# marco-conciatori-public/weed_instance_segmentation

Measured on AMD Instinct MI355X. Metric: images/sec at 1024x1024 bs=8 per GPU (Mask2Former R50, 100 queries, fp32 forward-only), higher is better.
Workload: dtype f32

## Files before the change

include/wm2f.h:

```cpp
#ifndef WM2F_H
#define WM2F_H

#include <stdint.h>

#ifdef __cplusplus
extern "C" {
#endif

#define WM2F_VERSION 100

#define WM2F_F32 0
#define WM2F_BF16 1
#define WM2F_I32 2
#define WM2F_U8 3
#define WM2F_U16 4
#define WM2F_I64 5

#define WM2F_OK 0
#define WM2F_EINVAL (-1)
#define WM2F_EUNSUPPORTED (-2)
#define WM2F_ELAUNCH (-3)

#define WM2F_MAX_LEVELS 8

int wm2f_version(void);
const char* wm2f_last_error(void);

int wm2f_msdeform_fwd(const void* value, const void* loc, const void* attn_w, void* out,
                      const int32_t* level_hw, int B, int S, int Q, int heads, int D, int L, int P,
                      int dtype, void* stream);

int wm2f_msdeform_bwd(const void* value, const void* loc, const void* attn_w, const void* grad_out,
                      void* grad_value, void* grad_loc, void* grad_attn_w,
                      const int32_t* level_hw, int B, int S, int Q, int heads, int D, int L, int P,
                      int dtype, void* stream);

int64_t wm2f_msdeform_bwd_det_workspace(const int32_t* level_hw, int B, int S, int heads, int D, int L);
int wm2f_msdeform_bwd_det(const void* value, const void* loc, const void* attn_w, const void* grad_out,
                          void* grad_value, void* grad_loc, void* grad_attn_w, void* workspace,
                          const int32_t* level_hw, int B, int S, int Q, int heads, int D, int L, int P, int dtype,
                          void* stream);

int wm2f_msdeform_rows_fwd(const void* value, const void* rows, void* out, const int32_t* level_hw, int B, int S, int Q,
                           int heads, int D, int L, int P, int dtype, void* stream);
int wm2f_msdeform_rows_bwd(const void* value, const void* rows, const void* grad_out, void* grad_value, void* grad_rows,
                           const int32_t* level_hw, int B, int S, int Q, int heads, int D, int L, int P, int dtype,
                           void* stream);

int wm2f_msdeform_fused_fwd(const void* value, const void* offsets, const void* logits, const void* ref,
                            void* out, const int32_t* level_hw, int B, int S, int Q, int heads, int D,
                            int L, int P, int dtype, void* stream);

int wm2f_msdeform_fused_packed_fwd(const void* value, const void* packed, void* out,
                                   const int32_t* level_hw, int B, int S, int Q, int heads, int D, int L,
                                   int P, int dtype, int margin, void* stream);

int wm2f_msdeform_fused_lanes_fwd(const void* value, const void* lanes, void* out, const int32_t* level_hw, int B, int S,
                                  int Q, int heads, int D, int L, int P, int dtype, int head_major, void* stream);

int wm2f_msdeform_fwd_v(const void* value, const void* a, const void* b, const void* ref, void* out,
                        const int32_t* level_hw, int B, int S, int Q, int heads, int D, int L, int P,
                        int dtype, int fused, int variant, int margin, void* stream);

int wm2f_mask_einsum_bf16_fwd(const void* emb, const void* pix_pixel_major, void* out, int B, int Q, int C,
                              int HW, void* stream);

int64_t wm2f_mask_einsum_bf16_bwd_workspace(int B, int Q, int C, int HW);
int wm2f_mask_einsum_bf16_bwd(const void* emb, const void* pix, const void* grad_out, void* g_emb, void* g_pix,
                              void* workspace, int B, int Q, int C, int HW, void* stream);
int wm2f_nchw_to_pixel_major_bf16(const void* src, void* dst, int B, int C, int HW, void* stream);

int wm2f_mask_einsum_fwd(const void* emb, const void* pix, void* out, int B, int Q, int C, int HW,
                         int dtype, void* stream);

int wm2f_mask_einsum_attn_mask_fwd(const void* emb, const void* pix, void* mask, void* row_open, int B, int Q, int C,
                                   int HW, int dtype, void* stream);

int64_t wm2f_mask_einsum_bwd_workspace(int B, int Q, int C, int HW);
int wm2f_mask_einsum_bwd(const void* emb, const void* pix, const void* grad_out, void* g_emb, void* g_pix,
                         void* workspace, int B, int Q, int C, int HW, int dtype, void* stream);

int wm2f_attn_mask_build(const void* logits, void* mask, void* row_open, int B, int Q, int H, int W,
                         int Hn, int Wn, void* stream);

int64_t wm2f_masked_xattn_workspace(int B, int heads, int Q, int N, int D);
int wm2f_masked_xattn_fwd(const void* q, const void* k, const void* v, const void* mask,
                          const void* row_open, void* out, void* lse, void* workspace,
                          int B, int heads, int Q, int N, int D, int dtype, void* stream);

int wm2f_masked_xattn_bf16_fwd(const void* q, const void* k, const void* v, const void* mask, const void* row_open,
                               void* out, void* lse, void* workspace, int B, int heads, int Q, int N, int D, void* stream);

int64_t wm2f_masked_xattn_bwd_workspace(int B, int heads, int Q, int N, int D);
int wm2f_masked_xattn_bwd(const void* q, const void* k, const void* v, const void* mask,
                          const void* row_open, const void* out, const void* lse, const void* grad_out,
                          void* grad_q, void* grad_k, void* grad_v, void* workspace,
                          int B, int heads, int Q, int N, int D, int dtype, void* stream);

int wm2f_masked_xattn_bf16_bwd(const void* q, const void* k, const void* v, const void* mask, const void* row_open,
                               const void* out, const void* lse, const void* grad_out, void* grad_q, void* grad_k,
                               void* grad_v, void* workspace, int B, int heads, int Q, int N, int D, void* stream);

#define WM2F_K2_UNSUPPORTED 0
#define WM2F_K2_FWD_GENERAL 1
#define WM2F_K2_FWD_FULL 2
#define WM2F_K2_BF16_FWD 3
#define WM2F_K2_BWD_GENERAL 4
#define WM2F_K2_BWD_FULL 5
#define WM2F_K2_BF16_BWD 6
int wm2f_masked_xattn_route(int B, int heads, int Q, int N, int D, int dtype, int backward, int mask_aligned, int* route);

int wm2f_swin_window_attn_fwd(const void* q, const void* k, const void* v, const void* k_pad, const void* v_pad,
                              const void* bias_table, void* out, int B, int H, int W, int heads, int D, int ws, int shift,
                              int dtype, void* stream);

int wm2f_swin_window_attn_train_fwd(const void* q, const void* k, const void* v, const void* k_pad, const void* v_pad,
                                    const void* bias_table, void* out, void* lse, int B, int H, int W, int heads, int D, int ws,
                                    int shift, int dtype, void* stream);
int64_t wm2f_swin_window_attn_bwd_workspace(int B, int H, int W, int heads, int D, int ws);
int wm2f_swin_window_attn_bwd(const void* q, const void* k, const void* v, const void* k_pad, const void* v_pad,
                              const void* bias_table, const void* lse, const void* grad_out, void* grad_q, void* grad_k,
                              void* grad_v, void* grad_k_pad, void* grad_v_pad, void* grad_bias_table, void* workspace, int B,
                              int H, int W, int heads, int D, int ws, int shift, int dtype, void* stream);

int64_t wm2f_matcher_workspace(int NL, int B, int Q, int P, int Tsum);
int wm2f_matcher_cost(const void* mask_logits, const void* class_logits, const void* tgt_masks,
                      int tgt_dtype, const int32_t* tgt_offset, const void* tgt_classes,
                      const void* points, void* cost, void* workspace, int NL, int B, int Q, int C1,
                      int h, int w, int Ht, int Wt, int P, int Tmax, float w_class, float w_mask,
                      float w_dice, void* stream);
int wm2f_matcher_cost_levels(const void* const* mask_levels, const void* class_logits, const void* tgt_masks,
                             int tgt_dtype, const int32_t* tgt_offset, const void* tgt_classes,
                             const void* points, void* cost, void* workspace, int NL, int B, int Q, int C1, int h,
                             int w, int Ht, int Wt, int P, int Tmax, float w_class, float w_mask, float w_dice,
                             void* stream);

int wm2f_lsa_batched(const void* cost, const void* counts, void* rows, void* cols, int problems, int B, int Q, int Tmax, int Tcap,
                     void* stream);

int wm2f_point_sample_fwd(const void* feat, int feat_dtype, const void* pts, const void* map_index,
                          void* out, int M, int H, int W, int P, void* stream);
int wm2f_point_sample_bwd(const void* grad_out, const void* pts, const void* map_index, void* grad_feat,
                          int M, int H, int W, int P, void* stream);

int wm2f_add_broadcast(const void* a, const void* p, void* out, int B, int64_t n, void* stream);
int wm2f_bias_act(const void* x, const void* bias, const void* residual, void* y, int N, int C, int HW,
                  int relu, void* stream);
int wm2f_add_layernorm(const void* x, const void* residual, const void* gamma, const void* beta,
                       const void* pos, void* out, void* out_plus_pos, int64_t rows, int C,
                       int64_t pos_rows, float eps, void* stream);
int64_t wm2f_add_layernorm_train_workspace(int64_t rows);
int wm2f_add_layernorm_train_fwd(const void* x, int x_dtype, const void* residual, const void* gamma, const void* beta,
                                 const void* pos, void* y, void* y_bf16, void* y_plus_pos, int yp_dtype, void* stats,
                                 int64_t rows, int C, int64_t pos_rows, float eps, float clamp, void* stream);
int wm2f_add_layernorm_train_bwd(const void* x, int x_dtype, const void* residual, const void* gamma, const void* stats,
                                 const void* grad_y, const void* grad_y_bf16, const void* grad_y_plus_pos, int gyp_dtype,
                                 void* grad_sum, void* grad_x, void* grad_gamma, void* grad_beta, void* workspace,
                                 int64_t rows, int C, void* stream);
int wm2f_token_linear_fwd(const void* x, const void* w, const void* bias, const void* residual, const void* ln_gamma,
                          const void* ln_beta, const void* pos, void* out, void* out_plus_pos, int64_t M, int K, int N, int relu,
                          int64_t pos_rows, float eps, int out_group, void* stream);

int wm2f_token_linear_split_weight(const void* w, void* w_split, int N, int K, void* stream);
int wm2f_token_linear_split_fwd(const void* x, const void* w_split, const void* bias, const void* residual, const void* ln_gamma,
                                const void* ln_beta, const void* pos, void* out, void* out_plus_pos, int64_t M, int K, int N,
                                int relu, int64_t pos_rows, float eps, int out_group, void* stream);

int wm2f_conv1x1_split_fwd(const void* x, const void* w_split, const void* bias, const void* residual, void* out, int B, int K,
                           int N, int Hi, int Wi, int stride, int relu, int config, void* stream);
int wm2f_conv1x1_split_config(int N, int P, int B, int n_cu);

int wm2f_conv3x3_split_fwd(const void* x, const void* w_split, const void* bias, void* out, int B, int Cin, int N, int Hi,
                           int Wi, int stride, int relu, int config, void* stream);
int wm2f_conv3x3_split_config(int N, int P, int B, int n_cu);

int wm2f_stem7x7_pool_fwd(const void* x, const void* w_split, const void* bias, void* out, int B, int Cin, int N, int Hi,
                          int Wi, int grid, void* stream);

int64_t wm2f_token_wgrad_workspace(int64_t M, int N, int K);
int wm2f_token_wgrad_bf16(const void* dy, const void* x, void* dw, void* db, void* workspace, int64_t M, int N, int K,
                          void* stream);
int wm2f_token_wgrad_f32(const void* dy, const void* x, void* dw, void* db, void* workspace, int64_t M, int N, int K,
                         void* stream);
int wm2f_tokens_to_nchw(const void* tokens, void* out, int B, int S, int C, int start, int HW, void* stream);
int wm2f_group_norm_tokens(const void* x, const void* bias, const void* gamma, const void* beta, void* tokens,
                           void* stats_ws, int B, int C, int G, int HW, int S, int start, float eps, void* stream);
int wm2f_resize_bilinear(const void* x, void* y, int NC, int H, int W, int Ho, int Wo, void* stream);
int wm2f_resize_pyramid(const void* x, void* y2, void* y4, void* y8, int NC, int H, int W, void* stream);
int wm2f_bias_relu_maxpool(const void* x, const void* bias, void* y, int N, int C, int H, int W, void* stream);
int wm2f_group_norm_act(const void* x, const void* gamma, const void* beta, const void* up, void* y, void* stats_ws,
                        int B, int C, int G, int H, int W, int Hs, int Ws, float eps, int relu, void* stream);

int wm2f_select_top_points(const void* score, const void* pts, void* out, int rows, int n, int k, int out_row_points,
                           void* stream);

int wm2f_point_sample_levels_fwd(const void* const* level_maps, int n_levels, const void* pts, const int32_t* index,
                                 void* out, int M, int H, int W, int P, int neg_abs, void* stream);
int wm2f_point_sample_levels_bwd(const void* grad_out, const void* pts, const int32_t* index,
                                 void* const* level_grads, int n_levels, int M, int H, int W, int P, void* stream);
int wm2f_point_sample_levels_bwd_unique(const void* grad_out, const void* pts, const int32_t* index,
                                        void* const* level_grads, int n_levels, int M, int H, int W, int P, void* stream);
int wm2f_mask_loss_rows_fwd(const void* logits, const void* labels, void* sums, void* bce_mean, void* dice,
                            int R, int P, void* stream);
int wm2f_mask_loss_rows_bwd(const void* logits, const void* labels, const void* sums, const void* g_bce,
                            const void* g_dice, void* grad, int R, int P, void* stream);

int wm2f_instance_scores(const void* mask_logits, const int32_t* qidx, void* sum_sig, void* cnt, int B, int Q,
                         int K, int h, int w, int gh, int gw, void* stream);
int wm2f_instance_any(const void* mask_logits, const int32_t* qidx, const uint8_t* cand, int32_t* any_out, int B,
                      int Q, int K, int h, int w, int gh, int gw, int Ho, int Wo, void* stream);
int wm2f_instance_segmentation(const void* mask_logits, const int32_t* kept_q, const int32_t* n_kept,
                               void* segmentation, int B, int Q, int K, int h, int w, int gh, int gw, int Ho,
                               int Wo, void* stream);
int wm2f_instance_maps(const void* image_logits, const int32_t* kept_q, int n, void* maps, int h, int w, int gh,
                       int gw, int Ho, int Wo, void* stream);

int wm2f_semantic_scores(const void* mask_logits, const void* class_probs, void* scores, int B, int Q, int C, int h,
                         int w, int gh, int gw, void* stream);
int wm2f_semantic_resize_argmax(const void* scores, const int32_t* rows, int nrows, void* segmentation,
                                void* out_scores, int C, int gh, int gw, int Ho, int Wo, void* stream);
int wm2f_panoptic_probs(const void* mask_logits, const int32_t* kept_q, const int32_t* n_kept, void* probs, int B,
                        int Q, int K, int h, int w, int gh, int gw, void* stream);
int wm2f_panoptic_segments(const void* probs, const int32_t* rows, const int32_t* n_kept, const void* scores,
                           int32_t* segmentation, int32_t* counts, int nrows, int K, int gh, int gw, int Ho, int Wo,
                           float mask_threshold, void* stream);
int wm2f_panoptic_relabel(int32_t* segmentation, const int32_t* rows, const int32_t* table, int nrows, int K,
                          int64_t n_pixels, void* stream);

int wm2f_labelmap_to_masks(const int32_t* label_map, const int32_t* ids, uint8_t* masks, int64_t n_pixels, int T,
                           void* stream);

int wm2f_labelmap_pair_counts(const void* pred_map, int pred_dtype, const void* gt_map, int gt_dtype,
                              const int32_t* gt_ids, const int32_t* n_ids, int32_t* hist, int B, int64_t n_pixels, int P,
                              int G, void* stream);
int64_t wm2f_mask_pair_counts_workspace(int D, int G, int64_t n_pixels);
int wm2f_mask_pair_counts(const uint8_t* det_masks, const uint8_t* gt_masks, int32_t* inter, int32_t* det_area,
                          int32_t* gt_area, void* workspace, int D, int G, int64_t n_pixels, void* stream);
int wm2f_coco_match(const int32_t* inter, const int32_t* det_area, const int32_t* gt_area, const int32_t* det_label,
                    const int32_t* gt_label, const int32_t* det_order, const int32_t* n_det, const int32_t* n_gt,
                    const double* iou_thresholds, const double* area_ranges, int32_t* det_rank, uint8_t* det_matched,
                    uint8_t* det_ignored, uint8_t* gt_ignored, int B, int D, int G, int T, int A, int max_det,
                    void* stream);
int wm2f_coco_match_min(const int32_t* inter, const int32_t* det_area, const int32_t* gt_area, const int32_t* inter2,
                        const int32_t* det_area2, const int32_t* gt_area2, const int32_t* det_label,
                        const int32_t* gt_label, const int32_t* det_order, const int32_t* n_det, const int32_t* n_gt,
                        const double* iou_thresholds, const double* area_ranges, int32_t* det_rank,
                        uint8_t* det_matched, uint8_t* det_ignored, uint8_t* gt_ignored, int B, int D, int G, int T,
                        int A, int max_det, void* stream);

int wm2f_labelmap_instance_stats(const void* map, int dtype, const int32_t* ids, const int32_t* n_ids, int64_t* stats,
                                 int B, int H, int W, int N, void* stream);

int64_t wm2f_labelmap_boundary_workspace(int B, int H, int W);
int wm2f_labelmap_boundary(const void* map, int dtype, int32_t* out, void* workspace, int B, int H, int W, int d,
                           void* stream);

int wm2f_panoptic_match(const int32_t* hist, const int32_t* pred_label, const int32_t* gt_label, const int32_t* n_pred,
                        const int32_t* n_gt, int32_t* gt_match, double* gt_iou, uint8_t* pred_state, int B, int P, int G,
                        int void_as_background, void* stream);
int wm2f_semantic_confusion(const void* pred, int pred_dtype, const void* gt, int gt_dtype, const int32_t* gt_ids,
                            const int32_t* gt_cls, const int32_t* n_ids, int64_t* conf, int64_t* n_out_of_range, int B,
                            int64_t n_pixels, int G, int C, int ignore_index, int background_label, void* stream);

int wm2f_labelmap_overlay(const uint8_t* image, const void* map, int dtype, const int32_t* ids, const int32_t* n_ids,
                          const uint8_t* rgba, const int32_t* order, uint32_t default_rgba, int inner, int outer,
                          uint8_t* out, int B, int H, int W, int N, void* stream);

#define WM2F_PRE_MAX_IMAGES 32
#define WM2F_PRE_MAX_SIDE 16384
#define WM2F_PRE_DESC_LEN 12
#define WM2F_LAB_DESC_LEN 7
int wm2f_resize_normalize_u8(const uint8_t* images, int64_t images_bytes, const int64_t* desc, const int32_t* tables,
                             int64_t n_table, const float* lut, uint8_t* workspace, int64_t workspace_bytes,
                             float* pixel_values, int64_t* pixel_mask, int B, int Hp, int Wp, void* stream);
int wm2f_resize_nearest_labels(const void* maps, int dtype, int64_t n_map_elems, const int64_t* desc,
                               const int32_t* tables, int64_t n_table, int32_t* out, uint8_t* present, int B, int Hp,
                               int Wp, int ignore_index, void* stream);

#define WM2F_AUG_MAX_VIRTUAL 65536
#define WM2F_AUG_PRE_DESC_LEN 16
#define WM2F_AUG_LAB_DESC_LEN 12
int wm2f_augment_resize_normalize_u8(const uint8_t* images, int64_t images_bytes, const int64_t* desc,
                                     const int32_t* tables, int64_t n_table, const float* lut, float* pixel_values,
                                     int64_t* pixel_mask, int B, int Hp, int Wp, void* stream);
int wm2f_augment_nearest_labels(const void* maps, int dtype, int64_t n_map_elems, const int64_t* desc,
                                const int32_t* tables, int64_t n_table, int32_t* out, uint8_t* present, int B, int Hp,
                                int Wp, int ignore_index, void* stream);

#define WM2F_PHOTO_BRIGHTNESS 0
#define WM2F_PHOTO_CONTRAST 1
#define WM2F_PHOTO_SATURATION 2
#define WM2F_PHOTO_HUE 3
#define WM2F_PHOTO_DESC_LEN 12
int64_t wm2f_photometric_workspace(int B);
int wm2f_photometric_u8(uint8_t* images, int64_t images_bytes, const int64_t* desc, void* workspace, int B, void* stream);

#define WM2F_CCL_VALUE 0
#define WM2F_CCL_BINARY 1
#define WM2F_CCL_RGB 2
#define WM2F_CCL_MAX_COLORS 16
int64_t wm2f_ccl_workspace(int H, int W);
int wm2f_ccl_label(const void* src, int mode, int src_dtype, int src_H, int src_W, const int32_t* ty, const int32_t* tx,
                   const uint8_t* colors, int n_colors, int H, int W, void* workspace, int32_t* count, void* stream);
int wm2f_ccl_keys(const void* workspace, int n, int H, int W, int64_t* keys, void* stream);
int wm2f_ccl_paint(void* workspace, const int64_t* order, int n, int H, int W, int skip_255, int background, int32_t* out,
                   int32_t* comp_class, void* stream);
int wm2f_resize_nearest(const void* src, int elem_bytes, int src_H, int src_W, const int32_t* ty, const int32_t* tx,
                        void* dst, int H, int W, void* stream);

#define WM2F_POLY_MAX_SIDE 16384
#define WM2F_POLY_MAX_COORD (1 << 24)
int64_t wm2f_poly_workspace(int H, int W, int n_verts);
int wm2f_poly_fill(int32_t* out, int H, int W, const int32_t* verts, int n_verts, const int32_t* contour_offsets,
                   int n_contours, const int32_t* call_offsets, const int32_t* values, const int32_t* call_row0,
                   const int32_t* item_offsets, int n_calls, int n_items, void* workspace, void* stream);

#define WM2F_RLE_MAX_IDS 1024
int64_t wm2f_rle_workspace(int B, int H, int W, int N, int order);
int wm2f_labelmap_toggle_counts(const void* map, int dtype, int32_t* counts, int32_t* out_of_range, void* workspace,
                                int B, int H, int W, int N, int order, void* stream);
int wm2f_labelmap_toggles(const void* map, int dtype, const int32_t* offsets, int32_t* positions, void* workspace, int B,
                          int H, int W, int N, int order, void* stream);
int64_t wm2f_rle_paint_workspace(int B, int H, int W);
int wm2f_rle_paint(int32_t* out, const int32_t* runs, int R, int32_t* status, void* workspace, int B, int H, int W,
                   int order, void* stream);

int64_t wm2f_trace_workspace(int B, int H, int W, int N);
int64_t wm2f_trace_edge_workspace(int64_t E);
int wm2f_trace_rounds(int64_t E);
int wm2f_trace_count(const void* map, int dtype, int32_t* counts, void* workspace, int B, int H, int W, int N,
                     void* stream);
int wm2f_trace_link(const void* map, int dtype, const void* workspace, void* edge_workspace, int E, int B, int H, int W,
                    int N, void* stream);
int wm2f_trace_rank(void* edge_workspace, int E, void* stream);
int wm2f_trace_flags(const void* edge_workspace, int32_t* flag, int32_t* lead, int E, int H, int W, int coords,
                     int simplify, void* stream);
int wm2f_trace_loops(const void* map, int dtype, const void* edge_workspace, const int32_t* lead_prefix,
                     int64_t* loop_key, int32_t* loop_len, int E, int n_loops, int B, int H, int W, int N, void* stream);
int wm2f_trace_scatter(const void* edge_workspace, const int32_t* flag, const int32_t* lead_prefix,
                       const int32_t* loop_place, const int32_t* loop_base, int32_t* flag_sorted, int32_t* edge_sorted,
                       int32_t* term_sorted, int E, int n_loops, int H, int W, void* stream);
int wm2f_trace_emit(const void* edge_workspace, const int32_t* flag_sorted, const int32_t* edge_sorted,
                    const int32_t* flag_prefix, int32_t* points, int E, int P, int H, int W, int coords, void* stream);

#define WM2F_TILE_MAX_SIDE 16384
#define WM2F_TILE_MAX_IDS 256
#define WM2F_TILE_MAX_TILES 1024
#define WM2F_TILE_MAX_PAIRS 16384
int64_t wm2f_tile_merge_workspace(int T, int N, int P);
int wm2f_tile_pair_counts(const void* tiles, int dtype, const int32_t* n_ids, const int32_t* pairs, int32_t* hist, int T,
                          int th, int tw, int N, int P, void* stream);
int wm2f_tile_owned_counts(const void* tiles, int dtype, const int32_t* n_ids, const int32_t* geom, int32_t* owned, int T,
                           int th, int tw, int N, void* stream);
int wm2f_tile_link(const int32_t* hist, const int32_t* pairs, const int32_t* labels, const int32_t* n_ids,
                   const int32_t* owned, int32_t* remap, int32_t* n_merged, void* workspace, int T, int N, int P, int num,
                   int den, void* stream);
int wm2f_tile_compose(const void* tiles, int dtype, const int32_t* n_ids, const int32_t* geom, const int32_t* remap,
                      int32_t* out, int T, int th, int tw, int N, int H, int W, void* stream);

#ifdef __cplusplus
}
#endif
#endif
```

weed_instance_segmentation_amd/_lib.py:

```python
from __future__ import annotations

import ctypes
import os
from ctypes import POINTER, c_char_p, c_float, c_int, c_int32, c_int64, c_void_p

HERE = os.path.dirname(os.path.abspath(__file__))
LIB_PATH = os.path.join(HERE, "libwm2f.so")
PROF_LIB_PATH = os.path.join(HERE, "libwm2f_prof.so")
if os.environ.get("WM2F_PROF_LIB"):
    PROF_LIB_PATH = os.environ["WM2F_PROF_LIB"]

WM2F_F32 = 0
WM2F_BF16 = 1
WM2F_I32 = 2
WM2F_U8 = 3
WM2F_U16 = 4
WM2F_I64 = 5
WM2F_CCL_VALUE, WM2F_CCL_BINARY, WM2F_CCL_RGB = 0, 1, 2
WM2F_CCL_MAX_COLORS = 16
WM2F_POLY_MAX_SIDE = 16384
WM2F_POLY_MAX_COORD = 1 << 24
WM2F_RLE_MAX_IDS = 1024
WM2F_AUG_MAX_VIRTUAL = 65536
WM2F_TILE_MAX_SIDE, WM2F_TILE_MAX_IDS, WM2F_TILE_MAX_TILES, WM2F_TILE_MAX_PAIRS = 16384, 256, 1024, 16384
WM2F_AUG_PRE_DESC_LEN, WM2F_AUG_LAB_DESC_LEN = 16, 12
WM2F_PHOTO_BRIGHTNESS, WM2F_PHOTO_CONTRAST, WM2F_PHOTO_SATURATION, WM2F_PHOTO_HUE = 0, 1, 2, 3
WM2F_PHOTO_DESC_LEN = 12
(WM2F_K2_UNSUPPORTED, WM2F_K2_FWD_GENERAL, WM2F_K2_FWD_FULL, WM2F_K2_BF16_FWD, WM2F_K2_BWD_GENERAL, WM2F_K2_BWD_FULL,
 WM2F_K2_BF16_BWD) = range(7)
WM2F_OK, WM2F_EINVAL, WM2F_EUNSUPPORTED, WM2F_ELAUNCH = 0, -1, -2, -3

_P = c_void_p
_I = c_int
_HOST_I32 = POINTER(c_int32)

SIGNATURES = {
    "wm2f_version": (c_int, []),
    "wm2f_last_error": (c_char_p, []),
    "wm2f_msdeform_fwd": (c_int, [_P, _P, _P, _P, _HOST_I32, _I, _I, _I, _I, _I, _I, _I, _I, _P]),
    "wm2f_msdeform_bwd": (c_int, [_P, _P, _P, _P, _P, _P, _P, _HOST_I32, _I, _I, _I, _I, _I, _I, _I, _I, _P]),
    "wm2f_msdeform_rows_fwd": (c_int, [_P, _P, _P, _HOST_I32, _I, _I, _I, _I, _I, _I, _I, _I, _P]),
    "wm2f_msdeform_rows_bwd": (c_int, [_P, _P, _P, _P, _P, _HOST_I32, _I, _I, _I, _I, _I, _I, _I, _I, _P]),
    "wm2f_msdeform_bwd_det_workspace": (c_int64, [_HOST_I32, _I, _I, _I, _I, _I]),
    "wm2f_msdeform_bwd_det": (c_int, [_P, _P, _P, _P, _P, _P, _P, _P, _HOST_I32, _I, _I, _I, _I, _I, _I, _I, _I, _P]),
    "wm2f_msdeform_fused_fwd": (c_int, [_P, _P, _P, _P, _P, _HOST_I32, _I, _I, _I, _I, _I, _I, _I, _I, _P]),
    "wm2f_msdeform_fused_packed_fwd": (c_int, [_P, _P, _P, _HOST_I32, _I, _I, _I, _I, _I, _I, _I, _I, _I, _P]),
    "wm2f_msdeform_fused_lanes_fwd": (c_int, [_P, _P, _P, _HOST_I32, _I, _I, _I, _I, _I, _I, _I, _I, _I, _P]),
    "wm2f_msdeform_fwd_v": (c_int, [_P, _P, _P, _P, _P, _HOST_I32, _I, _I, _I, _I, _I, _I, _I, _I, _I, _I, _I, _P]),
    "wm2f_select_top_points": (c_int, [_P, _P, _P, _I, _I, _I, _I, _P]),
    "wm2f_point_sample_levels_fwd": (c_int, [POINTER(c_void_p), _I, _P, _P, _P, _I, _I, _I, _I, _I, _P]),
    "wm2f_point_sample_levels_bwd": (c_int, [_P, _P, _P, POINTER(c_void_p), _I, _I, _I, _I, _I, _P]),
    "wm2f_point_sample_levels_bwd_unique": (c_int, [_P, _P, _P, POINTER(c_void_p), _I, _I, _I, _I, _I, _P]),
    "wm2f_mask_loss_rows_fwd": (c_int, [_P, _P, _P, _P, _P, _I, _I, _P]),
    "wm2f_mask_loss_rows_bwd": (c_int, [_P, _P, _P, _P, _P, _P, _I, _I, _P]),
    "wm2f_labelmap_to_masks": (c_int, [_P, _P, _P, c_int64, _I, _P]),
    "wm2f_instance_scores": (c_int, [_P, _P, _P, _P, _I, _I, _I, _I, _I, _I, _I, _P]),
    "wm2f_instance_any": (c_int, [_P, _P, _P, _P, _I, _I, _I, _I, _I, _I, _I, _I, _I, _P]),
    "wm2f_instance_segmentation": (c_int, [_P, _P, _P, _P, _I, _I, _I, _I, _I, _I, _I, _I, _I, _P]),
    "wm2f_instance_maps": (c_int, [_P, _P, _I, _P, _I, _I, _I, _I, _I, _I, _P]),
    "wm2f_semantic_scores": (c_int, [_P, _P, _P, _I, _I, _I, _I, _I, _I, _I, _P]),
    "wm2f_semantic_resize_argmax": (c_int, [_P, _P, _I, _P, _P, _I, _I, _I, _I, _I, _P]),
    "wm2f_panoptic_probs": (c_int, [_P, _P, _P, _P, _I, _I, _I, _I, _I, _I, _I, _P]),
    "wm2f_panoptic_segments": (c_int, [_P, _P, _P, _P, _P, _P, _I, _I, _I, _I, _I, _I, c_float, _P]),
    "wm2f_panoptic_relabel": (c_int, [_P, _P, _P, _I, _I, c_int64, _P]),
    "wm2f_mask_einsum_bf16_fwd": (c_int, [_P, _P, _P, _I, _I, _I, _I, _P]),
    "wm2f_nchw_to_pixel_major_bf16": (c_int, [_P, _P, _I, _I, _I, _P]),
    "wm2f_mask_einsum_fwd": (c_int, [_P, _P, _P, _I, _I, _I, _I, _I, _P]),
    "wm2f_mask_einsum_attn_mask_fwd": (c_int, [_P, _P, _P, _P, _I, _I, _I, _I, _I, _P]),
    "wm2f_mask_einsum_bf16_bwd_workspace": (c_int64, [_I, _I, _I, _I]),
    "wm2f_mask_einsum_bf16_bwd": (c_int, [_P, _P, _P, _P, _P, _P, _I, _I, _I, _I, _P]),
    "wm2f_mask_einsum_bwd_workspace": (c_int64, [_I, _I, _I, _I]),
    "wm2f_mask_einsum_bwd": (c_int, [_P, _P, _P, _P, _P, _P, _I, _I, _I, _I, _I, _P]),
    "wm2f_attn_mask_build": (c_int, [_P, _P, _P, _I, _I, _I, _I, _I, _I, _P]),
    "wm2f_masked_xattn_workspace": (c_int64, [_I, _I, _I, _I, _I]),
    "wm2f_masked_xattn_fwd": (c_int, [_P, _P, _P, _P, _P, _P, _P, _P, _I, _I, _I, _I, _I, _I, _P]),
    "wm2f_masked_xattn_route": (c_int, [_I, _I, _I, _I, _I, _I, _I, _I, _HOST_I32]),
    "wm2f_masked_xattn_bf16_fwd": (c_int, [_P, _P, _P, _P, _P, _P, _P, _P, _I, _I, _I, _I, _I, _P]),
    "wm2f_masked_xattn_bf16_bwd": (c_int, [_P, _P, _P, _P, _P, _P, _P, _P, _P, _P, _P, _P, _I, _I, _I, _I, _I, _P]),
    "wm2f_masked_xattn_bwd_workspace": (c_int64, [_I, _I, _I, _I, _I]),
    "wm2f_masked_xattn_bwd": (c_int, [_P, _P, _P, _P, _P, _P, _P, _P, _P, _P, _P, _P, _I, _I, _I, _I, _I, _I, _P]),
    "wm2f_swin_window_attn_fwd": (c_int, [_P, _P, _P, _P, _P, _P, _P, _I, _I, _I, _I, _I, _I, _I, _I, _P]),
    "wm2f_swin_window_attn_train_fwd": (c_int, [_P, _P, _P, _P, _P, _P, _P, _P, _I, _I, _I, _I, _I, _I, _I, _I, _P]),
    "wm2f_swin_window_attn_bwd_workspace": (c_int64, [_I, _I, _I, _I, _I, _I]),
    "wm2f_swin_window_attn_bwd": (c_int, [_P] * 15 + [_I] * 8 + [_P]),
    "wm2f_matcher_workspace": (c_int64, [_I, _I, _I, _I, _I]),
    "wm2f_matcher_cost": (c_int, [_P, _P, _P, _I, _HOST_I32, _P, _P, _P, _P, _I, _I, _I, _I, _I, _I, _I, _I, _I, _I,
                                  c_float, c_float, c_float, _P]),
    "wm2f_matcher_cost_levels": (c_int, [POINTER(c_void_p), _P, _P, _I, _HOST_I32, _P, _P, _P, _P, _I, _I, _I, _I, _I, _I, _I,
                                         _I, _I, _I, c_float, c_float, c_float, _P]),
    "wm2f_lsa_batched": (c_int, [_P, _P, _P, _P, _I, _I, _I, _I, _I, _P]),
    "wm2f_add_broadcast": (c_int, [_P, _P, _P, _I, c_int64, _P]),
    "wm2f_bias_act": (c_int, [_P, _P, _P, _P, _I, _I, _I, _I, _P]),
    "wm2f_add_layernorm": (c_int, [_P, _P, _P, _P, _P, _P, _P, c_int64, _I, c_int64, c_float, _P]),
    "wm2f_add_layernorm_train_workspace": (c_int64, [c_int64]),
    "wm2f_add_layernorm_train_fwd": (c_int, [_P, _I, _P, _P, _P, _P, _P, _P, _P, _I, _P, c_int64, _I, c_int64, c_float, c_float, _P]),
    "wm2f_add_layernorm_train_bwd": (c_int, [_P, _I, _P, _P, _P, _P, _P, _P, _I, _P, _P, _P, _P, _P, c_int64, _I, _P]),
    "wm2f_token_linear_fwd": (c_int, [_P, _P, _P, _P, _P, _P, _P, _P, _P, c_int64, _I, _I, _I, c_int64, c_float, _I, _P]),
    "wm2f_token_linear_split_weight": (c_int, [_P, _P, _I, _I, _P]),
    "wm2f_token_linear_split_fwd": (c_int, [_P, _P, _P, _P, _P, _P, _P, _P, _P, c_int64, _I, _I, _I, c_int64, c_float, _I, _P]),
    "wm2f_conv1x1_split_config": (c_int, [_I, _I, _I, _I]),
    "wm2f_conv1x1_split_fwd": (c_int, [_P, _P, _P, _P, _P, _I, _I, _I, _I, _I, _I, _I, _I, _P]),
    "wm2f_conv3x3_split_config": (c_int, [_I, _I, _I, _I]),
    "wm2f_conv3x3_split_fwd": (c_int, [_P, _P, _P, _P, _I, _I, _I, _I, _I, _I, _I, _I, _P]),
    "wm2f_stem7x7_pool_fwd": (c_int, [_P, _P, _P, _P, _I, _I, _I, _I, _I, _I, _P]),
    "wm2f_token_wgrad_workspace": (c_int64, [c_int64, _I, _I]),
    "wm2f_token_wgrad_bf16": (c_int, [_P, _P, _P, _P, _P, c_int64, _I, _I, _P]),
    "wm2f_token_wgrad_f32": (c_int, [_P, _P, _P, _P, _P, c_int64, _I, _I, _P]),
    "wm2f_tokens_to_nchw": (c_int, [_P, _P, _I, _I, _I, _I, _I, _P]),
    "wm2f_group_norm_tokens": (c_int, [_P, _P, _P, _P, _P, _P, _I, _I, _I, _I, _I, _I, c_float, _P]),
    "wm2f_resize_bilinear": (c_int, [_P, _P, _I, _I, _I, _I, _I, _P]),
    "wm2f_resize_pyramid": (c_int, [_P, _P, _P, _P, _I, _I, _I, _P]),
    "wm2f_bias_relu_maxpool": (c_int, [_P, _P, _P, _I, _I, _I, _I, _P]),
    "wm2f_group_norm_act": (c_int, [_P, _P, _P, _P, _P, _P, _I, _I, _I, _I, _I, _I, _I, c_float, _I, _P]),
    "wm2f_point_sample_fwd": (c_int, [_P, _I, _P, _P, _P, _I, _I, _I, _I, _P]),
    "wm2f_point_sample_bwd": (c_int, [_P, _P, _P, _P, _I, _I, _I, _I, _P]),
    "wm2f_labelmap_pair_counts": (c_int, [_P, _I, _P, _I, _P, _P, _P, _I, c_int64, _I, _I, _P]),
    "wm2f_mask_pair_counts_workspace": (c_int64, [_I, _I, c_int64]),
    "wm2f_mask_pair_counts": (c_int, [_P, _P, _P, _P, _P, _P, _I, _I, c_int64, _P]),
    "wm2f_coco_match": (c_int, [_P] * 14 + [_I, _I, _I, _I, _I, _I, _P]),
    "wm2f_coco_match_min": (c_int, [_P] * 17 + [_I, _I, _I, _I, _I, _I, _P]),
    "wm2f_labelmap_boundary_workspace": (c_int64, [_I, _I, _I]),
    "wm2f_labelmap_boundary": (c_int, [_P, _I, _P, _P, _I, _I, _I, _I, _P]),
    "wm2f_labelmap_instance_stats": (c_int, [_P, _I, _P, _P, _P, _I, _I, _I, _I, _P]),
    "wm2f_panoptic_match": (c_int, [_P] * 8 + [_I, _I, _I, _I, _P]),
    "wm2f_semantic_confusion": (c_int, [_P, _I, _P, _I, _P, _P, _P, _P, _P, _I, c_int64, _I, _I, _I, _I, _P]),
    "wm2f_labelmap_overlay": (c_int, [_P, _P, _I, _P, _P, _P, _P, ctypes.c_uint32, _I, _I, _P, _I, _I, _I, _I, _P]),
    "wm2f_resize_normalize_u8": (c_int, [_P, c_int64, POINTER(c_int64), _P, c_int64, _P, _P, c_int64, _P, _P, _I, _I, _I,
                                         _P]),
    "wm2f_resize_nearest_labels": (c_int, [_P, _I, c_int64, POINTER(c_int64), _P, c_int64, _P, _P, _I, _I, _I, _I, _P]),
    "wm2f_augment_resize_normalize_u8": (c_int, [_P, c_int64, POINTER(c_int64), _P, c_int64, _P, _P, _P, _I, _I, _I, _P]),
    "wm2f_augment_nearest_labels": (c_int, [_P, _I, c_int64, POINTER(c_int64), _P, c_int64, _P, _P, _I, _I, _I, _I, _P]),
    "wm2f_photometric_workspace": (c_int64, [_I]),
    "wm2f_photometric_u8": (c_int, [_P, c_int64, POINTER(c_int64), _P, _I, _P]),
    "wm2f_ccl_workspace": (c_int64, [_I, _I]),
    "wm2f_ccl_label": (c_int, [_P, _I, _I, _I, _I, _P, _P, POINTER(ctypes.c_uint8), _I, _I, _I, _P, _P, _P]),
    "wm2f_ccl_keys": (c_int, [_P, _I, _I, _I, _P, _P]),
    "wm2f_ccl_paint": (c_int, [_P, _P, _I, _I, _I, _I, _I, _P, _P, _P]),
    "wm2f_resize_nearest": (c_int, [_P, _I, _I, _I, _P, _P, _P, _I, _I, _P]),
    "wm2f_poly_workspace": (c_int64, [_I, _I, _I]),
    "wm2f_poly_fill": (c_int, [_P, _I, _I, _P, _I, _P, _I, _P, _P, _P, _P, _I, _I, _P, _P]),
    "wm2f_rle_workspace": (c_int64, [_I, _I, _I, _I, _I]),
    "wm2f_labelmap_toggle_counts": (c_int, [_P, _I, _P, _P, _P, _I, _I, _I, _I, _I, _P]),
    "wm2f_labelmap_toggles": (c_int, [_P, _I, _P, _P, _P, _I, _I, _I, _I, _I, _P]),
    "wm2f_rle_paint_workspace": (c_int64, [_I, _I, _I]),
    "wm2f_rle_paint": (c_int, [_P, _P, _I, _P, _P, _I, _I, _I, _I, _P]),
    "wm2f_trace_workspace": (c_int64, [_I, _I, _I, _I]),
    "wm2f_trace_edge_workspace": (c_int64, [c_int64]),
    "wm2f_trace_rounds": (c_int, [c_int64]),
    "wm2f_trace_count": (c_int, [_P, _I, _P, _P, _I, _I, _I, _I, _P]),
    "wm2f_trace_link": (c_int, [_P, _I, _P, _P, _I, _I, _I, _I, _I, _P]),
    "wm2f_trace_rank": (c_int, [_P, _I, _P]),
    "wm2f_trace_flags": (c_int, [_P, _P, _P, _I, _I, _I, _I, _I, _P]),
    "wm2f_trace_loops": (c_int, [_P, _I, _P, _P, _P, _P, _I, _I, _I, _I, _I, _I, _P]),
    "wm2f_trace_scatter": (c_int, [_P, _P, _P, _P, _P, _P, _P, _P, _I, _I, _I, _I, _P]),
    "wm2f_trace_emit": (c_int, [_P, _P, _P, _P, _P, _I, _I, _I, _I, _I, _P]),
    "wm2f_tile_merge_workspace": (c_int64, [_I, _I, _I]),
    "wm2f_tile_pair_counts": (c_int, [_P, _I, _P, _P, _P, _I, _I, _I, _I, _I, _P]),
    "wm2f_tile_owned_counts": (c_int, [_P, _I, _P, _P, _P, _I, _I, _I, _I, _P]),
    "wm2f_tile_link": (c_int, [_P, _P, _P, _P, _P, _P, _P, _P, _I, _I, _I, _I, _I, _P]),
    "wm2f_tile_compose": (c_int, [_P, _I, _P, _P, _P, _P, _I, _I, _I, _I, _I, _I, _P]),
}

PROF_SIGNATURES = {"wm2f_debug_stamps": (c_int, [_P, c_int64])}

_lib = None


class Wm2fError(RuntimeError):
    pass


def use_profiling_library() -> ctypes.CDLL:
    global _lib
    if _lib is not None:
        raise Wm2fError("use_profiling_library() must come before the first kernel call")
    if not os.path.exists(PROF_LIB_PATH):
        raise Wm2fError(f"{PROF_LIB_PATH} not found: python -m weed_instance_segmentation_amd._build --prof")
    lib = ctypes.CDLL(PROF_LIB_PATH)
    for name, (res, args) in {**SIGNATURES, **PROF_SIGNATURES}.items():
        fn = getattr(lib, name)
        fn.restype, fn.argtypes = res, args
    _lib = lib
    return lib


def load() -> ctypes.CDLL:
    global _lib
    if _lib is None:
        if not os.path.exists(LIB_PATH):
            raise Wm2fError(
                f"{LIB_PATH} not found: build it with `python -m weed_instance_segmentation_amd._build` "
                "(hipcc, gfx950). There is no CPU or PyTorch fallback for the hot path.")
        lib = ctypes.CDLL(LIB_PATH)
        for name, (res, args) in SIGNATURES.items():
            fn = getattr(lib, name)
            fn.restype = res
            fn.argtypes = args
        _lib = lib
    return _lib


def check(rc: int, what: str) -> None:
    if rc != 0:
        msg = load().wm2f_last_error()
        raise Wm2fError(f"{what} failed (code {rc}): {msg.decode() if msg else '?'}")


def host_i32(values) -> ctypes.Array:
    flat = [int(v) for v in values]
    return (c_int32 * len(flat))(*flat)
```

weed_instance_segmentation_amd/csrc/conv1x1_split.hip:

```cpp
#include "common.h"

namespace wm2f {
namespace {

using f32x4 = __attribute__((ext_vector_type(4))) float;
using f32x8 = __attribute__((ext_vector_type(8))) float;
using bf16x8 = __attribute__((ext_vector_type(8))) __bf16;
typedef __attribute__((address_space(3))) void* lds_ptr_t;

constexpr int kWaves = 8;
constexpr int kThreads = kWaves * 64;
constexpr int kCT = 2;
constexpr int kKStep = 32;
constexpr int kFrag = 1024;
constexpr unsigned kOob = 0x80000000u;
constexpr float kBf16Max = 3.38953139e38f;

enum : int { kRaw = 0, kBias = 1, kBiasRelu = 2, kBiasResRelu = 3 };

__device__ __forceinline__ void split3(const f32x8 x, bf16x8& h, bf16x8& m, bf16x8& l) {
  f32x8 xc;
#pragma unroll
  for (int i = 0; i < 8; ++i) xc[i] = __builtin_amdgcn_fmed3f(x[i], -kBf16Max, kBf16Max);
  h = __builtin_convertvector(xc, bf16x8);
  const f32x8 r1 = x - __builtin_convertvector(h, f32x8);
  m = __builtin_convertvector(r1, bf16x8);
  const f32x8 r2 = r1 - __builtin_convertvector(m, f32x8);
  l = __builtin_convertvector(r2, bf16x8);
}

struct C1Args {
  const float *x, *bias, *residual;
  const void* ws;
  float* out;
  int K, N;
  int Hi, Wi, Wo, P, stride;
};

__device__ __forceinline__ void c1_barrier() {
  asm volatile("s_waitcnt vmcnt(0)" ::: "memory");
  __builtin_amdgcn_s_barrier();
  asm volatile("" ::: "memory");
}

template <int NRT, int WN, int EPI>
__global__ __launch_bounds__(kThreads) void conv1x1_split_kernel(C1Args a) {
  extern __shared__ __attribute__((aligned(16))) unsigned char smem[];
  constexpr int kRowTiles = WN * NRT;
  constexpr int kPanelBytes = kRowTiles * 3 * kFrag;
  constexpr int kPieces = kRowTiles * 3;
  constexpr int kPT = (kWaves / WN) * kCT * 16;
  const int tid = threadIdx.x, lane = tid & 63, wave = __builtin_amdgcn_readfirstlane(tid >> 6);
  const int wn = wave % WN, wp = wave / WN;
  const int g = lane >> 4, j = lane & 15;
  const int nb = blockIdx.x, b = blockIdx.z;
  const int n_wg = nb * kRowTiles * 16;
  const int p_w = blockIdx.y * kPT + wp * kCT * 16;
  const int n_ks = a.K / kKStep;
  const int HWi = a.Hi * a.Wi;

  const __amdgpu_buffer_rsrc_t w_rs = __builtin_amdgcn_make_buffer_rsrc((void*)a.ws, 0, a.N * a.K * 6, 0x00020000);
  const __amdgpu_buffer_rsrc_t x_rs =
      __builtin_amdgcn_make_buffer_rsrc((void*)(a.x + (int64_t)b * a.K * HWi), 0, a.K * HWi * 4, 0x00020000);

  unsigned xo[kCT];
#pragma unroll
  for (int c = 0; c < kCT; ++c) {
    const int p = p_w + c * 16 + j;
    const int ho = p / a.Wo, wo = p - ho * a.Wo;
    xo[c] = p < a.P ? (unsigned)(((8 * g) * HWi + a.stride * (ho * a.Wi + wo)) * 4) : kOob;
  }
  const unsigned ch_bytes = (unsigned)HWi * 4;

  f32x8 xr[kCT];
  auto issue = [&](int ks) {
    unsigned char* dst = smem + (ks & 1) * kPanelBytes;
    const int src = (ks * (a.N / 16) + n_wg / 16) * 3 * kFrag;
    for (int f = wave; f < kPieces; f += kWaves)
      __builtin_amdgcn_raw_ptr_buffer_load_lds(w_rs, (lds_ptr_t)(dst + f * kFrag), 16, lane * 16, src + f * kFrag, 0, 0);
    const unsigned kb = (unsigned)(ks * kKStep) * ch_bytes;
#pragma unroll
    for (int c = 0; c < kCT; ++c) {
      const unsigned o = xo[c] == kOob ? kOob : xo[c] + kb;
#pragma unroll
      for (int i = 0; i < 8; ++i)
        xr[c][i] = __builtin_bit_cast(float, __builtin_amdgcn_raw_buffer_load_b32(x_rs, o, i * ch_bytes, 0));
    }
  };

  issue(0);
  c1_barrier();

  f32x4 acc[NRT][kCT];
#pragma unroll
  for (int rt = 0; rt < NRT; ++rt)
#pragma unroll
    for (int c = 0; c < kCT; ++c) acc[rt][c] = (f32x4){0.f, 0.f, 0.f, 0.f};

  for (int ks = 0; ks < n_ks; ++ks) {
    bf16x8 bh[kCT], bm[kCT], bl[kCT];
#pragma unroll
    for (int c = 0; c < kCT; ++c) split3(xr[c], bh[c], bm[c], bl[c]);
    if (ks + 1 < n_ks) issue(ks + 1);

    const unsigned char* panel = smem + (ks & 1) * kPanelBytes + wn * NRT * 3 * kFrag;
    auto read_a = [&](bf16x8 (&dst)[3], int rt) {
#pragma unroll
      for (int p = 0; p < 3; ++p) dst[p] = *reinterpret_cast<const bf16x8*>(panel + (rt * 3 + p) * kFrag + lane * 16);
    };
    auto six = [&](f32x4 acc_in, const bf16x8 (&av)[3], int cc) {
      f32x4 c = __builtin_amdgcn_mfma_f32_16x16x32_bf16(av[1], bm[cc], (f32x4){0.f, 0.f, 0.f, 0.f}, 0, 0, 0);
      c = __builtin_amdgcn_mfma_f32_16x16x32_bf16(av[2], bh[cc], c, 0, 0, 0);
      c = __builtin_amdgcn_mfma_f32_16x16x32_bf16(av[0], bl[cc], c, 0, 0, 0);
      c = __builtin_amdgcn_mfma_f32_16x16x32_bf16(av[1], bh[cc], c, 0, 0, 0);
      c = __builtin_amdgcn_mfma_f32_16x16x32_bf16(av[0], bm[cc], c, 0, 0, 0);
      return acc_in + __builtin_amdgcn_mfma_f32_16x16x32_bf16(av[0], bh[cc], c, 0, 0, 0);
    };
    bf16x8 av[2][3];
    read_a(av[0], 0);
#pragma unroll
    for (int rt = 0; rt < NRT; ++rt) {
      if (rt + 1 < NRT) read_a(av[(rt + 1) & 1], rt + 1);
      __builtin_amdgcn_sched_barrier(0);
      acc[rt][0] = six(acc[rt][0], av[rt & 1], 0);
      acc[rt][1] = six(acc[rt][1], av[rt & 1], 1);
      __builtin_amdgcn_sched_barrier(0);
    }
    c1_barrier();
  }

  const int64_t img = (int64_t)b * a.N * a.P;
  const __amdgpu_buffer_rsrc_t o_rs = __builtin_amdgcn_make_buffer_rsrc((void*)(a.out + img), 0, a.N * a.P * 4, 0x00020000);
  __amdgpu_buffer_rsrc_t r_rs = o_rs;
  if (EPI == kBiasResRelu) r_rs = __builtin_amdgcn_make_buffer_rsrc((void*)(a.residual + img), 0, a.N * a.P * 4, 0x00020000);
  const int n0 = n_wg + wn * NRT * 16 + 4 * g;
#pragma unroll
  for (int rt = 0; rt < NRT; ++rt) {
    float bv[4] = {0.f, 0.f, 0.f, 0.f};
    if (EPI != kRaw) {
#pragma unroll
      for (int e = 0; e < 4; ++e) bv[e] = a.bias[n0 + rt * 16 + e];
    }
#pragma unroll
    for (int c = 0; c < kCT; ++c) {
      const int p = p_w + c * 16 + j;
      const unsigned ro = p < a.P ? (unsigned)(((n0 + rt * 16) * a.P + p) * 4) : kOob;
      const unsigned rs = (unsigned)a.P * 4;
      float rv[4] = {0.f, 0.f, 0.f, 0.f};
      if (EPI == kBiasResRelu) {
#pragma unroll
        for (int e = 0; e < 4; ++e) rv[e] = __builtin_bit_cast(float, __builtin_amdgcn_raw_buffer_load_b32(r_rs, ro, e * rs, 0));
      }
#pragma unroll
      for (int e = 0; e < 4; ++e) {
        float v = acc[rt][c][e];
        if (EPI != kRaw) v += bv[e];
        if (EPI == kBiasResRelu) v += rv[e];
        if (EPI == kBiasRelu || EPI == kBiasResRelu) v = v < 0.f ? 0.f : v;
        __builtin_amdgcn_raw_buffer_store_b32(__builtin_bit_cast(unsigned, v), o_rs, ro, e * rs, 0);
      }
    }
  }
}

struct Cfg {
  int nrt, wn;
};
constexpr Cfg kCfg[] = {{16, 1}, {8, 2}, {4, 4}, {8, 1}, {4, 1}};
constexpr int kNumCfg = sizeof(kCfg) / sizeof(kCfg[0]);

template <int NRT, int WN>
void (*pick_epi(int epi))(C1Args) {
  switch (epi) {
    case kRaw: return conv1x1_split_kernel<NRT, WN, kRaw>;
    case kBias: return conv1x1_split_kernel<NRT, WN, kBias>;
    case kBiasRelu: return conv1x1_split_kernel<NRT, WN, kBiasRelu>;
    default: return conv1x1_split_kernel<NRT, WN, kBiasResRelu>;
  }
}

void (*pick_kernel(int ci, int epi))(C1Args) {
  switch (ci) {
    case 0: return pick_epi<16, 1>(epi);
    case 1: return pick_epi<8, 2>(epi);
    case 2: return pick_epi<4, 4>(epi);
    case 3: return pick_epi<8, 1>(epi);
    default: return pick_epi<4, 1>(epi);
  }
}

int choose_cfg(int N, int P, int B, int n_cu) {
  int best = -1;
  int64_t best_cost = 0;
  for (int i = 0; i < kNumCfg; ++i) {
    const int nt = kCfg[i].wn * kCfg[i].nrt * 16, pt = (kWaves / kCfg[i].wn) * kCT * 16;
    if (N % nt) continue;
    const int64_t wgs = (int64_t)(N / nt) * ceil_div(P, pt) * B;
    const int64_t cost = ceil_div64(wgs, n_cu) * (kCfg[i].nrt + 4);
    if (best < 0 || cost < best_cost) best = i, best_cost = cost;
  }
  return best;
}

int cu_count(int* n_cu) {
  int dev = 0;
  if (hipGetDevice(&dev) != hipSuccess) return -1;
  static int cached[64] = {0};
  if (dev < 0 || dev >= 64) return -1;
  if (cached[dev] == 0) {
    hipDeviceProp_t prop;
    if (hipGetDeviceProperties(&prop, dev) != hipSuccess) return -1;
    cached[dev] = prop.multiProcessorCount;
  }
  *n_cu = cached[dev];
  return 0;
}

}
}

using namespace wm2f;

extern "C" int wm2f_conv1x1_split_config(int N, int P, int B, int n_cu) {
  if (N <= 0 || P <= 0 || B <= 0 || n_cu <= 0) return -1;
  return choose_cfg(N, P, B, n_cu);
}

extern "C" int wm2f_conv1x1_split_fwd(const void* x, const void* w_split, const void* bias, const void* residual, void* out,
                                      int B, int K, int N, int Hi, int Wi, int stride, int relu, int config, void* stream) {
  const char* who = "wm2f_conv1x1_split_fwd";
  WM2F_REQUIRE(x && w_split && out, "%s: null pointer", who);
  WM2F_REQUIRE(B > 0 && K > 0 && N > 0 && Hi > 0 && Wi > 0, "%s: non-positive size", who);
  WM2F_REQUIRE(K % kKStep == 0 && N % 64 == 0, "%s: K = %d must be a multiple of %d and N = %d of 64", who, K, kKStep, N);
  WM2F_REQUIRE(stride == 1 || stride == 2, "%s: stride %d (1 and 2 are built)", who, stride);
  const int Ho = (Hi - 1) / stride + 1, Wo = (Wi - 1) / stride + 1;
  const int64_t P = (int64_t)Ho * Wo;
  WM2F_REQUIRE((int64_t)K * Hi * Wi * 4 < (1ll << 31) && (int64_t)N * P * 4 < (1ll << 31),
               "%s: one image of x / out must stay below 2 GiB (32-bit buffer offsets)", who);
  WM2F_REQUIRE((int64_t)N * K * 6 < (1ll << 31), "%s: the split weight must stay below 2 GiB", who);
  WM2F_REQUIRE(!residual || (bias && relu), "%s: the residual epilogue is bias + residual + ReLU", who);
  WM2F_REQUIRE(!relu || bias, "%s: the ReLU epilogues carry a bias", who);
  int n_cu = 0;
  if (cu_count(&n_cu) != 0) {
    set_error("%s: cannot query the device", who);
    return WM2F_ELAUNCH;
  }
  WM2F_REQUIRE(config >= -1 && config < kNumCfg, "%s: configuration %d out of range", who, config);
  const int ci = config >= 0 ? config : choose_cfg(N, (int)P, B, n_cu);
  WM2F_REQUIRE(ci >= 0 && N % (kCfg[ci].wn * kCfg[ci].nrt * 16) == 0, "%s: no configuration %d for N = %d", who, ci, N);
  const int epi = residual ? kBiasResRelu : (relu ? kBiasRelu : (bias ? kBias : kRaw));
  const int nt = kCfg[ci].wn * kCfg[ci].nrt * 16, pt = (kWaves / kCfg[ci].wn) * kCT * 16;
  C1Args a;
  a.x = (const float*)x;
  a.ws = w_split;
  a.bias = (const float*)bias;
  a.residual = (const float*)residual;
  a.out = (float*)out;
  a.K = K;
  a.N = N;
  a.Hi = Hi;
  a.Wi = Wi;
  a.Wo = Wo;
  a.P = (int)P;
  a.stride = stride;
  const size_t lds = (size_t)2 * (nt / 16) * 3 * kFrag;
  void (*kfn)(C1Args) = pick_kernel(ci, epi);
  hipError_t e = hipFuncSetAttribute((const void*)kfn, hipFuncAttributeMaxDynamicSharedMemorySize, (int)lds);
  if (e != hipSuccess) {
    set_error("%s: cannot raise dynamic LDS to %zu: %s", who, lds, hipGetErrorString(e));
    return WM2F_ELAUNCH;
  }
  hipLaunchKernelGGL(kfn, dim3(N / nt, ceil_div((int)P, pt), B), dim3(kThreads), lds, (hipStream_t)stream, a);
  WM2F_CHECK_LAUNCH(who);
  return WM2F_OK;
}
```

weed_instance_segmentation_amd/csrc/conv3x3_split.hip:

```cpp
#include "common.h"

namespace wm2f {
namespace {

using f32x4 = __attribute__((ext_vector_type(4))) float;
using f32x8 = __attribute__((ext_vector_type(8))) float;
using bf16x8 = __attribute__((ext_vector_type(8))) __bf16;
typedef __attribute__((address_space(3))) void* lds_ptr_t;

constexpr int kWaves = 8;
constexpr int kThreads = kWaves * 64;
constexpr int kCT = 2;
constexpr int kKStep = 32;
constexpr int kFrag = 1024;
constexpr unsigned kOob = 0x80000000u;
constexpr float kBf16Max = 3.38953139e38f;

enum : int { kRaw = 0, kBias = 1, kBiasRelu = 2 };

__device__ __forceinline__ f32x8 widen(const bf16x8 v) {
  using u32x4 = __attribute__((ext_vector_type(4))) unsigned;
  const u32x4 w = __builtin_bit_cast(u32x4, v);
  f32x8 r;
#pragma unroll
  for (int i = 0; i < 4; ++i) {
    r[2 * i] = __builtin_bit_cast(float, w[i] << 16);
    r[2 * i + 1] = __builtin_bit_cast(float, w[i] & 0xffff0000u);
  }
  return r;
}

__device__ __forceinline__ void split3(const f32x8 x, bf16x8& h, bf16x8& m, bf16x8& l) {
  f32x8 xc;
#pragma unroll
  for (int i = 0; i < 8; ++i) xc[i] = __builtin_amdgcn_fmed3f(x[i], -kBf16Max, kBf16Max);
  h = __builtin_convertvector(xc, bf16x8);
  const f32x8 r1 = x - widen(h);
  m = __builtin_convertvector(r1, bf16x8);
  const f32x8 r2 = r1 - widen(m);
  l = __builtin_convertvector(r2, bf16x8);
}

struct C3Args {
  const float *x, *bias;
  const void* ws;
  float* out;
  int Cin, N;
  int Hi, Wi, Wo, P, stride;
};

__device__ __forceinline__ void c3_barrier() {
  asm volatile("s_waitcnt vmcnt(0)" ::: "memory");
  __builtin_amdgcn_s_barrier();
  asm volatile("" ::: "memory");
}

template <int NRT, int WN, int EPI>
__global__ __launch_bounds__(kThreads) void conv3x3_split_kernel(C3Args a) {
  extern __shared__ __attribute__((aligned(16))) unsigned char smem[];
  constexpr int kRowTiles = WN * NRT;
  constexpr int kPanelBytes = kRowTiles * 3 * kFrag;
  constexpr int kPieces = kRowTiles * 3;
  constexpr int kPT = (kWaves / WN) * kCT * 16;
  const int tid = threadIdx.x, lane = tid & 63, wave = __builtin_amdgcn_readfirstlane(tid >> 6);
  const int wn = wave % WN, wp = wave / WN;
  const int g = lane >> 4, j = lane & 15;
  const int nb = blockIdx.x, b = blockIdx.z;
  const int n_wg = nb * kRowTiles * 16;
  const int p_w = blockIdx.y * kPT + wp * kCT * 16;
  const int n_cb = a.Cin / kKStep;
  const int n_ks = 9 * n_cb;
  const int HWi = a.Hi * a.Wi;

  const __amdgpu_buffer_rsrc_t w_rs = __builtin_amdgcn_make_buffer_rsrc((void*)a.ws, 0, a.N * 9 * a.Cin * 6, 0x00020000);
  const __amdgpu_buffer_rsrc_t x_rs =
      __builtin_amdgcn_make_buffer_rsrc((void*)(a.x + (int64_t)b * a.Cin * HWi), 0, a.Cin * HWi * 4, 0x00020000);

  int xo[kCT];
  unsigned tap_ok[kCT];
#pragma unroll
  for (int c = 0; c < kCT; ++c) {
    const int p = p_w + c * 16 + j;
    const int ho = p / a.Wo, wo = p - ho * a.Wo;
    const int hi = a.stride * ho - 1, wi = a.stride * wo - 1;
    xo[c] = ((8 * g) * HWi + hi * a.Wi + wi) * 4;
    unsigned m = 0;
    if (p < a.P) {
#pragma unroll
      for (int dy = 0; dy < 3; ++dy)
#pragma unroll
        for (int dx = 0; dx < 3; ++dx)
          if ((unsigned)(hi + dy) < (unsigned)a.Hi && (unsigned)(wi + dx) < (unsigned)a.Wi) m |= 1u << (3 * dy + dx);
    }
    tap_ok[c] = m;
  }
  const unsigned ch_bytes = (unsigned)HWi * 4;

  f32x8 xr[kCT];
  auto issue = [&](int it) {
    const int cb = it / 9, tap = it - 9 * cb;
    const int dy = tap / 3, dx = tap - 3 * dy;
    unsigned char* dst = smem + (it & 1) * kPanelBytes;
    const int src = ((tap * n_cb + cb) * (a.N / 16) + n_wg / 16) * 3 * kFrag;
    for (int f = wave; f < kPieces; f += kWaves)
      __builtin_amdgcn_raw_ptr_buffer_load_lds(w_rs, (lds_ptr_t)(dst + f * kFrag), 16, lane * 16, src + f * kFrag, 0, 0);
    const int kb = (cb * kKStep * HWi + dy * a.Wi + dx) * 4;
#pragma unroll
    for (int c = 0; c < kCT; ++c) {
      const unsigned o = (tap_ok[c] >> tap) & 1u ? (unsigned)(xo[c] + kb) : kOob;
#pragma unroll
      for (int i = 0; i < 8; ++i)
        xr[c][i] = __builtin_bit_cast(float, __builtin_amdgcn_raw_buffer_load_b32(x_rs, o, i * ch_bytes, 0));
    }
  };

  issue(0);
  c3_barrier();

  f32x4 acc[NRT][kCT];
#pragma unroll
  for (int rt = 0; rt < NRT; ++rt)
#pragma unroll
    for (int c = 0; c < kCT; ++c) acc[rt][c] = (f32x4){0.f, 0.f, 0.f, 0.f};

  for (int it = 0; it < n_ks; ++it) {
    bf16x8 bh[kCT], bm[kCT], bl[kCT];
#pragma unroll
    for (int c = 0; c < kCT; ++c) split3(xr[c], bh[c], bm[c], bl[c]);
    if (it + 1 < n_ks) issue(it + 1);

    const unsigned char* panel = smem + (it & 1) * kPanelBytes + wn * NRT * 3 * kFrag;
    auto read_a = [&](bf16x8 (&dst)[3], int rt) {
#pragma unroll
      for (int p = 0; p < 3; ++p) dst[p] = *reinterpret_cast<const bf16x8*>(panel + (rt * 3 + p) * kFrag + lane * 16);
    };
    auto six = [&](f32x4 acc_in, const bf16x8 (&av)[3], int cc) {
      f32x4 c = __builtin_amdgcn_mfma_f32_16x16x32_bf16(av[1], bm[cc], (f32x4){0.f, 0.f, 0.f, 0.f}, 0, 0, 0);
      c = __builtin_amdgcn_mfma_f32_16x16x32_bf16(av[2], bh[cc], c, 0, 0, 0);
      c = __builtin_amdgcn_mfma_f32_16x16x32_bf16(av[0], bl[cc], c, 0, 0, 0);
      c = __builtin_amdgcn_mfma_f32_16x16x32_bf16(av[1], bh[cc], c, 0, 0, 0);
      c = __builtin_amdgcn_mfma_f32_16x16x32_bf16(av[0], bm[cc], c, 0, 0, 0);
      return acc_in + __builtin_amdgcn_mfma_f32_16x16x32_bf16(av[0], bh[cc], c, 0, 0, 0);
    };
    bf16x8 av[2][3];
    read_a(av[0], 0);
#pragma unroll
    for (int rt = 0; rt < NRT; ++rt) {
      if (rt + 1 < NRT) read_a(av[(rt + 1) & 1], rt + 1);
      __builtin_amdgcn_sched_barrier(0);
      acc[rt][0] = six(acc[rt][0], av[rt & 1], 0);
      acc[rt][1] = six(acc[rt][1], av[rt & 1], 1);
      __builtin_amdgcn_sched_barrier(0);
    }
    c3_barrier();
  }

  const int64_t img = (int64_t)b * a.N * a.P;
  const __amdgpu_buffer_rsrc_t o_rs = __builtin_amdgcn_make_buffer_rsrc((void*)(a.out + img), 0, a.N * a.P * 4, 0x00020000);
  const int n0 = n_wg + wn * NRT * 16 + 4 * g;
#pragma unroll
  for (int rt = 0; rt < NRT; ++rt) {
    float bv[4] = {0.f, 0.f, 0.f, 0.f};
    if (EPI != kRaw) {
#pragma unroll
      for (int e = 0; e < 4; ++e) bv[e] = a.bias[n0 + rt * 16 + e];
    }
#pragma unroll
    for (int c = 0; c < kCT; ++c) {
      const int p = p_w + c * 16 + j;
      const unsigned ro = p < a.P ? (unsigned)(((n0 + rt * 16) * a.P + p) * 4) : kOob;
      const unsigned rs = (unsigned)a.P * 4;
#pragma unroll
      for (int e = 0; e < 4; ++e) {
        float v = acc[rt][c][e];
        if (EPI != kRaw) v += bv[e];
        if (EPI == kBiasRelu) v = v < 0.f ? 0.f : v;
        __builtin_amdgcn_raw_buffer_store_b32(__builtin_bit_cast(unsigned, v), o_rs, ro, e * rs, 0);
      }
    }
  }
}

struct Cfg {
  int nrt, wn;
};
constexpr Cfg kCfg[] = {{16, 1}, {8, 2}, {4, 4}, {8, 1}, {4, 1}};
constexpr int kNumCfg = sizeof(kCfg) / sizeof(kCfg[0]);

template <int NRT, int WN>
void (*pick_epi(int epi))(C3Args) {
  switch (epi) {
    case kRaw: return conv3x3_split_kernel<NRT, WN, kRaw>;
    case kBias: return conv3x3_split_kernel<NRT, WN, kBias>;
    default: return conv3x3_split_kernel<NRT, WN, kBiasRelu>;
  }
}

void (*pick_kernel(int ci, int epi))(C3Args) {
  switch (ci) {
    case 0: return pick_epi<16, 1>(epi);
    case 1: return pick_epi<8, 2>(epi);
    case 2: return pick_epi<4, 4>(epi);
    case 3: return pick_epi<8, 1>(epi);
    default: return pick_epi<4, 1>(epi);
  }
}

int choose_cfg(int N, int P, int B, int n_cu) {
  int best = -1;
  int64_t best_cost = 0;
  for (int i = 0; i < kNumCfg; ++i) {
    const int nt = kCfg[i].wn * kCfg[i].nrt * 16, pt = (kWaves / kCfg[i].wn) * kCT * 16;
    if (N % nt) continue;
    const int64_t wgs = (int64_t)(N / nt) * ceil_div(P, pt) * B;
    const int64_t cost = ceil_div64(wgs, n_cu) * (kCfg[i].nrt + 4);
    if (best < 0 || cost < best_cost || (cost == best_cost && kCfg[i].wn < kCfg[best].wn)) best = i, best_cost = cost;
  }
  return best;
}

int cu_count(int* n_cu) {
  int dev = 0;
  if (hipGetDevice(&dev) != hipSuccess) return -1;
  static int cached[64] = {0};
  if (dev < 0 || dev >= 64) return -1;
  if (cached[dev] == 0) {
    hipDeviceProp_t prop;
    if (hipGetDeviceProperties(&prop, dev) != hipSuccess) return -1;
    cached[dev] = prop.multiProcessorCount;
  }
  *n_cu = cached[dev];
  return 0;
}

}
}

using namespace wm2f;

extern "C" int wm2f_conv3x3_split_config(int N, int P, int B, int n_cu) {
  if (N <= 0 || P <= 0 || B <= 0 || n_cu <= 0) return -1;
  return choose_cfg(N, P, B, n_cu);
}

extern "C" int wm2f_conv3x3_split_fwd(const void* x, const void* w_split, const void* bias, void* out, int B, int Cin, int N,
                                      int Hi, int Wi, int stride, int relu, int config, void* stream) {
  const char* who = "wm2f_conv3x3_split_fwd";
  WM2F_REQUIRE(x && w_split && out, "%s: null pointer", who);
  WM2F_REQUIRE(B > 0 && Cin > 0 && N > 0 && Hi > 0 && Wi > 0, "%s: non-positive size", who);
  WM2F_REQUIRE(Cin % kKStep == 0 && N % 64 == 0, "%s: Cin = %d must be a multiple of %d and N = %d of 64", who, Cin, kKStep, N);
  WM2F_REQUIRE(stride == 1 || stride == 2, "%s: stride %d (1 and 2 are built)", who, stride);
  const int Ho = (Hi - 1) / stride + 1, Wo = (Wi - 1) / stride + 1;
  const int64_t P = (int64_t)Ho * Wo;
  WM2F_REQUIRE((int64_t)Cin * Hi * Wi * 4 < (1ll << 31) && (int64_t)N * P * 4 < (1ll << 31),
               "%s: one image of x / out must stay below 2 GiB (32-bit buffer offsets)", who);
  WM2F_REQUIRE((int64_t)N * 9 * Cin * 6 < (1ll << 31), "%s: the split weight must stay below 2 GiB", who);
  WM2F_REQUIRE(!relu || bias, "%s: the ReLU epilogue carries a bias", who);
  int n_cu = 0;
  if (cu_count(&n_cu) != 0) {
    set_error("%s: cannot query the device", who);
    return WM2F_ELAUNCH;
  }
  WM2F_REQUIRE(config >= -1 && config < kNumCfg, "%s: configuration %d out of range", who, config);
  const int ci = config >= 0 ? config : choose_cfg(N, (int)P, B, n_cu);
  WM2F_REQUIRE(ci >= 0 && N % (kCfg[ci].wn * kCfg[ci].nrt * 16) == 0, "%s: no configuration %d for N = %d", who, ci, N);
  const int epi = relu ? kBiasRelu : (bias ? kBias : kRaw);
  const int nt = kCfg[ci].wn * kCfg[ci].nrt * 16, pt = (kWaves / kCfg[ci].wn) * kCT * 16;
  C3Args a;
  a.x = (const float*)x;
  a.ws = w_split;
  a.bias = (const float*)bias;
  a.out = (float*)out;
  a.Cin = Cin;
  a.N = N;
  a.Hi = Hi;
  a.Wi = Wi;
  a.Wo = Wo;
  a.P = (int)P;
  a.stride = stride;
  const size_t lds = (size_t)2 * (nt / 16) * 3 * kFrag;
  void (*kfn)(C3Args) = pick_kernel(ci, epi);
  hipError_t e = hipFuncSetAttribute((const void*)kfn, hipFuncAttributeMaxDynamicSharedMemorySize, (int)lds);
  if (e != hipSuccess) {
    set_error("%s: cannot raise dynamic LDS to %zu: %s", who, lds, hipGetErrorString(e));
    return WM2F_ELAUNCH;
  }
  hipLaunchKernelGGL(kfn, dim3(N / nt, ceil_div((int)P, pt), B), dim3(kThreads), lds, (hipStream_t)stream, a);
  WM2F_CHECK_LAUNCH(who);
  return WM2F_OK;
}
```

weed_instance_segmentation_amd/ops/__init__.py:

```python
from __future__ import annotations

K1_BWD_DETERMINISTIC: bool | None = None

CONV1X1_SPLIT = True

CONV3X3_SPLIT = True

from .._lib import check
from ._core import KernelTimer, _p, _stream, set_kernel_timer
from .ccl import label_components, resize_nearest_tables
from .fused import (add_broadcast, bias_act_, bias_relu_maxpool, group_norm_act_, group_norm_tokens_, resize_bilinear,
                    resize_pyramid, tokens_to_nchw)
from .gemm import (conv1x1, conv1x1_applies, conv3x3, conv3x3_applies, linear_tokens, split_weight, split_weight_3x3,
                   split_weight_cached, split_weight_stem, stem_conv_pool, stem_conv_pool_applies, stem_weight_columns,
                   stem_weight_matrix, token_linear, token_linear_applies, token_wgrad, token_wgrad_applies)
from .k1 import (k1_bwd_deterministic, k1_lane_order, k1_lane_rows, k1_lanes_applies, k1_rows_applies, ms_deform_attn,
                 ms_deform_attn_bwd, ms_deform_attn_fused, ms_deform_attn_fused_lanes, ms_deform_attn_fused_packed,
                 ms_deform_attn_rows, ms_deform_attn_variant)
from .k2 import masked_xattn, masked_xattn_bf16_applies
from .k3 import (attn_mask_build, mask_einsum, mask_einsum_attn_mask, mask_einsum_bf16, mask_einsum_bf16_bwd,
                 mask_einsum_bf16_bwd_applies, mask_einsum_bwd, mask_einsum_bwd_applies, nchw_to_pixel_major_bf16)
from .labelmaps import (coco_match, coco_match_min, labelmap_boundary, labelmap_instance_stats, labelmap_pair_counts,
                        labelmap_to_masks, mask_pair_counts, panoptic_match, semantic_confusion_)
from .layernorm import add_layernorm, add_layernorm_train, add_layernorm_train_applies
from .loss import mask_loss_rows, point_sample, point_sample_levels, select_top_points
from .matcher import lsa_batched, matcher_cost
from .overlay import labelmap_overlay
from .polygons import fill_polygons
from .postprocess import (_GRID, instance_any, instance_maps, instance_scores, instance_segmentation, panoptic_probs,
                          panoptic_relabel_, panoptic_segments, semantic_resize_argmax, semantic_scores)
from .rle import labelmap_toggle_counts, labelmap_toggles, rle_paint_
from .trace import labelmap_trace
from .tiles import tile_compose, tile_link, tile_owned_counts, tile_pair_counts
from .preprocess import (augment_nearest_labels, augment_resize_normalize_u8, photometric_u8, resize_nearest_labels,
                         resize_normalize_u8)
from .swin import (SWIN_HEAD_DIMS, SWIN_WINDOW_SIZES, swin_window_attention, swin_window_attention_applies,
                   swin_window_attention_train)
```

weed_instance_segmentation_amd/ops/gemm.py:

```python
from __future__ import annotations

import weakref

import torch

from .._lib import load
from ._core import _launch, _p, _req
from .fused import bias_act_, bias_relu_maxpool


def token_linear_applies(x: torch.Tensor, weight: torch.Tensor) -> bool:
    N, K = weight.shape
    M = x.numel() // max(K, 1)
    return (x.is_cuda and x.dtype == torch.float32 and weight.dtype == torch.float32 and N in (256, 288, 512, 768, 1024)
            and K % 32 == 0 and x.shape[-1] == K and M * K * 4 < (1 << 31) and M * N * 4 < (1 << 31)
            and N * K * 6 < (1 << 31))


def split_weight(weight: torch.Tensor) -> torch.Tensor:
    weight = _req(weight, "weight")
    N, K = weight.shape
    ws = torch.empty(N * K * 6, device=weight.device, dtype=torch.uint8)
    _launch("wm2f_token_linear_split_weight", weight, _p(weight), _p(ws), N, K)
    return ws


def split_weight_cached(owner, name: str, weight: torch.Tensor, base: torch.Tensor | None = None,
                        tap_major: bool = False) -> torch.Tensor:
    ident = weight if base is None else base
    c = owner.__dict__.setdefault("_wm2f_split", {})
    key = (ident._version, weight.data_ptr(), weight.device, tuple(weight.shape))
    hit = c.get(name)
    if hit is None or hit[0]() is not ident or hit[1] != key:
        if not tap_major:
            ws = split_weight(weight)
        else:
            ws = split_weight_stem(weight) if tuple(weight.shape[2:]) == (7, 7) else split_weight_3x3(weight)
        hit = (weakref.ref(ident), key, ws)
        c[name] = hit
    return hit[2]


def split_weight_3x3(weight: torch.Tensor) -> torch.Tensor:
    N = int(weight.shape[0])
    return split_weight(weight.permute(0, 2, 3, 1).reshape(N, -1).contiguous())


def token_linear(x: torch.Tensor, weight: torch.Tensor, bias: torch.Tensor, relu: bool = False, residual: torch.Tensor | None = None,
                 ln: tuple | None = None, pos: torch.Tensor | None = None, out_group: int = 0, split: bool = True,
                 w_split: torch.Tensor | None = None):
    x, weight, bias = _req(x, "x"), _req(weight, "weight"), _req(bias, "bias")
    N, K = weight.shape
    if x.shape[-1] != K or bias.shape != (N,):
        raise ValueError(f"token_linear: x {tuple(x.shape)} weight {tuple(weight.shape)} bias {tuple(bias.shape)}")
    M = x.numel() // K
    if out_group and (out_group % 4 or N % out_group or ln is not None):
        raise ValueError("token_linear: out_group must divide N, be a multiple of 4 and exclude the LayerNorm epilogue")
    out = (torch.empty(N // out_group, *x.shape[:-1], out_group, device=x.device, dtype=torch.float32) if out_group
           else torch.empty(*x.shape[:-1], N, device=x.device, dtype=torch.float32))
    gamma = beta = None
    eps = 0.0
    if ln is not None:
        gamma, beta, eps = _req(ln[0], "gamma"), _req(ln[1], "beta"), float(ln[2])
    if residual is not None:
        residual = _req(residual, "residual")
        if residual.numel() != M * N:
            raise ValueError("token_linear: residual shape")
    out_pos, pos_rows = None, 0
    if pos is not None:
        pos = _req(pos, "pos")
        pos_rows = pos.numel() // N
        if M % pos_rows:
            raise ValueError("token_linear: pos rows do not divide the token count")
        out_pos = torch.empty_like(out)
    tag = f"token_linear_K{K}_N{N}" + ("_ln" if ln is not None else "")
    if split:
        if w_split is None:
            w_split = split_weight(weight)
        elif w_split.dtype != torch.uint8 or w_split.numel() != N * K * 6 or w_split.device != x.device:
            raise ValueError("token_linear: w_split is not split_weight(weight)")
        _launch("wm2f_token_linear_split_fwd", x, _p(x), _p(w_split), _p(bias), _p(residual), _p(gamma), _p(beta), _p(pos),
                _p(out), _p(out_pos), M, K, N, 1 if relu else 0, pos_rows, eps, int(out_group), tag=tag + "_split")
    else:
        _launch("wm2f_token_linear_fwd", x, _p(x), _p(weight), _p(bias), _p(residual), _p(gamma), _p(beta), _p(pos), _p(out),
                _p(out_pos), M, K, N, 1 if relu else 0, pos_rows, eps, int(out_group), tag=tag)
    return (out, out_pos) if pos is not None else out


def conv1x1_applies(x: torch.Tensor, weight: torch.Tensor, stride: int = 1) -> bool:
    if x.dim() != 4 or weight.dim() not in (2, 4) or (weight.dim() == 4 and weight.shape[2:] != (1, 1)):
        return False
    N, K = int(weight.shape[0]), int(weight.shape[1])
    _, C, H, W = x.shape
    Ho, Wo = (H - 1) // stride + 1, (W - 1) // stride + 1
    return (x.is_cuda and x.dtype == torch.float32 and weight.dtype == torch.float32 and C == K and K % 32 == 0
            and N % 64 == 0 and stride in (1, 2) and K * H * W * 4 < (1 << 31) and N * Ho * Wo * 4 < (1 << 31)
            and N * K * 6 < (1 << 31))


def conv1x1(x: torch.Tensor, weight: torch.Tensor, bias: torch.Tensor | None = None, residual: torch.Tensor | None = None,
            relu: bool = False, stride: int = 1, split: bool = True, w_split: torch.Tensor | None = None,
            config: int = -1) -> torch.Tensor:
    if residual is not None and (bias is None or not relu):
        raise ValueError("conv1x1: the residual epilogue is bias + residual + ReLU")
    if relu and bias is None:
        raise ValueError("conv1x1: the ReLU epilogues carry a bias")
    N, K = int(weight.shape[0]), int(weight.shape[1])
    if not split or not conv1x1_applies(x, weight, stride):
        w4 = weight if weight.dim() == 4 else weight.view(N, K, 1, 1)
        y = torch.nn.functional.conv2d(x, w4, None, stride)
        if bias is None:
            return y
        if (y.shape[-1] * y.shape[-2]) % 4 == 0:
            return bias_act_(y, bias, residual, relu)
        y = y + bias[None, :, None, None]
        if residual is not None:
            y = y + residual
        return torch.relu(y) if relu else y
    x = _req(x, "x")
    w2 = _req(weight.reshape(N, K), "weight")
    B, _, H, W = x.shape
    Ho, Wo = (H - 1) // stride + 1, (W - 1) // stride + 1
    if bias is not None:
        bias = _req(bias, "bias")
        if bias.shape != (N,):
            raise ValueError(f"conv1x1: bias {tuple(bias.shape)} for {N} channels")
    if residual is not None:
        residual = _req(residual, "residual")
        if residual.shape != (B, N, Ho, Wo):
            raise ValueError(f"conv1x1: residual {tuple(residual.shape)}, output ({B}, {N}, {Ho}, {Wo})")
    if w_split is None:
        w_split = split_weight(w2)
    elif w_split.dtype != torch.uint8 or w_split.numel() != N * K * 6 or w_split.device != x.device:
        raise ValueError("conv1x1: w_split is not split_weight(weight)")
    out = torch.empty(B, N, Ho, Wo, device=x.device, dtype=torch.float32)
    _launch("wm2f_conv1x1_split_fwd", x, _p(x), _p(w_split), _p(bias), _p(residual), _p(out), B, K, N, H, W, int(stride),
            1 if relu else 0, int(config), tag=f"conv1x1_K{K}_N{N}_P{Ho * Wo}")
    return out


def conv3x3_applies(x: torch.Tensor, weight: torch.Tensor, stride: int = 1) -> bool:
    if x.dim() != 4 or weight.dim() != 4 or tuple(weight.shape[2:]) != (3, 3):
        return False
    N, C = int(weight.shape[0]), int(weight.shape[1])
    _, K, H, W = x.shape
    Ho, Wo = (H - 1) // stride + 1, (W - 1) // stride + 1
    return (x.is_cuda and x.dtype == torch.float32 and weight.dtype == torch.float32 and C == K and K % 32 == 0
            and N % 64 == 0 and stride in (1, 2) and K * H * W * 4 < (1 << 31) and N * Ho * Wo * 4 < (1 << 31)
            and N * 9 * K * 6 < (1 << 31))


def conv3x3(x: torch.Tensor, weight: torch.Tensor, bias: torch.Tensor | None = None, relu: bool = False, stride: int = 1,
            split: bool = True, w_split: torch.Tensor | None = None, config: int = -1) -> torch.Tensor:
    if relu and bias is None:
        raise ValueError("conv3x3: the ReLU epilogue carries a bias")
    if not split or not conv3x3_applies(x, weight, stride):
        y = torch.nn.functional.conv2d(x, weight, None, stride, 1)
        if bias is None:
            return y
        if (y.shape[-1] * y.shape[-2]) % 4 == 0:
            return bias_act_(y, bias, None, relu)
        y = y + bias[None, :, None, None]
        return torch.relu(y) if relu else y
    x = _req(x, "x")
    N, Cin = int(weight.shape[0]), int(weight.shape[1])
    B, _, H, W = x.shape
    Ho, Wo = (H - 1) // stride + 1, (W - 1) // stride + 1
    if bias is not None:
        bias = _req(bias, "bias")
        if bias.shape != (N,):
            raise ValueError(f"conv3x3: bias {tuple(bias.shape)} for {N} channels")
    if w_split is None:
        w_split = split_weight_3x3(_req(weight, "weight"))
    elif w_split.dtype != torch.uint8 or w_split.numel() != N * 9 * Cin * 6 or w_split.device != x.device:
        raise ValueError("conv3x3: w_split is not split_weight_3x3(weight)")
    out = torch.empty(B, N, Ho, Wo, device=x.device, dtype=torch.float32)
    _launch("wm2f_conv3x3_split_fwd", x, _p(x), _p(w_split), _p(bias), _p(out), B, Cin, N, H, W, int(stride), 1 if relu else 0,
            int(config), tag=f"conv3x3_C{Cin}_N{N}_P{Ho * Wo}")
    return out


STEM_K = 160


def stem_weight_columns(cin: int) -> torch.Tensor:
    if cin not in (1, 2, 3):
        raise ValueError(f"stem_weight_columns: Cin = {cin} (1, 2 and 3 are built)")
    cols = torch.full((STEM_K,), -1, dtype=torch.long)
    rows = 7 * cin
    for G in range(min(rows, STEM_K // 8)):
        cols[8 * G:8 * G + 7] = torch.arange(7 * G, 7 * G + 7)
    if rows > STEM_K // 8:
        cols[7:8 * 7:8] = torch.arange(7 * 20, 7 * 21)
    return cols


def stem_weight_matrix(weight: torch.Tensor) -> torch.Tensor:
    N, cin = int(weight.shape[0]), int(weight.shape[1])
    cols = stem_weight_columns(cin).to(weight.device)
    flat = torch.cat([weight.reshape(N, -1), weight.new_zeros(N, 1)], 1)
    return flat[:, torch.where(cols < 0, torch.full_like(cols, 49 * cin), cols)].contiguous()


def split_weight_stem(weight: torch.Tensor) -> torch.Tensor:
    return split_weight(stem_weight_matrix(_req(weight, "weight")))


def stem_conv_pool_applies(x: torch.Tensor, weight: torch.Tensor) -> bool:
    if x.dim() != 4 or weight.dim() != 4 or tuple(weight.shape[2:]) != (7, 7):
        return False
    N, C = int(weight.shape[0]), int(weight.shape[1])
    _, K, H, W = x.shape
    Hp, Wp = ((H - 1) // 2) // 2 + 1, ((W - 1) // 2) // 2 + 1
    return (x.is_cuda and x.dtype == torch.float32 and weight.dtype == torch.float32 and C == K and C in (1, 2, 3)
            and N == 64 and H >= 1 and W >= 1 and K * H * W * 4 < (1 << 31) and N * Hp * Wp * 4 < (1 << 31))


def stem_conv_pool(x: torch.Tensor, weight: torch.Tensor, bias: torch.Tensor, w_split: torch.Tensor | None = None,
                   split: bool = True, grid: int = 0) -> torch.Tensor:
    if not split or not stem_conv_pool_applies(x, weight):
        y = torch.nn.functional.conv2d(x, weight, None, 2, 3)
        if y.is_cuda and y.dtype == torch.float32 and y.shape[-2] % 2 == 0 and y.shape[-1] % 8 == 0:
            return bias_relu_maxpool(y, bias)
        return torch.nn.functional.max_pool2d(torch.relu_(y.add_(bias[None, :, None, None])), 3, 2, 1)
    x, bias = _req(x, "x"), _req(bias, "bias")
    N, Cin = int(weight.shape[0]), int(weight.shape[1])
    B, _, H, W = x.shape
    if bias.shape != (N,):
        raise ValueError(f"stem_conv_pool: bias {tuple(bias.shape)} for {N} channels")
    if w_split is None:
        w_split = split_weight_stem(weight)
    elif w_split.dtype != torch.uint8 or w_split.numel() != N * STEM_K * 6 or w_split.device != x.device:
        raise ValueError("stem_conv_pool: w_split is not split_weight_stem(weight)")
    out = torch.empty(B, N, ((H - 1) // 2) // 2 + 1, ((W - 1) // 2) // 2 + 1, device=x.device, dtype=torch.float32)
    _launch("wm2f_stem7x7_pool_fwd", x, _p(x), _p(w_split), _p(bias), _p(out), B, Cin, N, H, W, int(grid), tag="stem7x7_pool")
    return out


def token_wgrad_applies(dy: torch.Tensor, x: torch.Tensor) -> bool:
    N, K = dy.shape[-1], x.shape[-1]
    M = x.numel() // max(K, 1)
    es = x.element_size()
    return (dy.is_cuda and x.is_cuda and dy.dtype == x.dtype and x.dtype in (torch.bfloat16, torch.float32) and N % 8 == 0
            and K % 8 == 0 and dy.numel() == M * N and M * N * es < 0x7fffffff and M * K * es < 0x7fffffff)


def token_wgrad(dy: torch.Tensor, x: torch.Tensor, want_bias: bool = True):
    if x.dtype not in (torch.bfloat16, torch.float32):
        raise TypeError(f"token_wgrad: {x.dtype}")
    dy, x = _req(dy, "dy", x.dtype), _req(x, "x", x.dtype)
    N, K = dy.shape[-1], x.shape[-1]
    M = x.numel() // K
    if dy.numel() != M * N:
        raise ValueError(f"token_wgrad: dy {tuple(dy.shape)} x {tuple(x.shape)}")
    dw = torch.empty(N, K, device=x.device, dtype=torch.float32)
    db = torch.empty(N, device=x.device, dtype=torch.float32) if want_bias else None
    bf = x.dtype == torch.bfloat16
    ws = torch.empty(max(16, int(load().wm2f_token_wgrad_workspace(M, N, K))), device=x.device, dtype=torch.uint8)
    _launch("wm2f_token_wgrad_bf16" if bf else "wm2f_token_wgrad_f32", x, _p(dy), _p(x), _p(dw), _p(db), _p(ws), M, N, K,
            tag=f"token_wgrad_{'bf16' if bf else 'f32'}_N{N}_K{K}", what="wm2f_token_wgrad")
    return dw, db


class _TokenLinear(torch.autograd.Function):

    @staticmethod
    def forward(ctx, x, weight, bias, bf16):
        cdt = torch.bfloat16 if bf16 else torch.float32
        xc, wc = x.to(cdt), weight.to(cdt)
        ctx.save_for_backward(xc, wc)
        ctx.x_dtype, ctx.has_bias, ctx.cdt = x.dtype, bias is not None, cdt
        return torch.nn.functional.linear(xc, wc, None if bias is None else bias.to(cdt))

    @staticmethod
    def backward(ctx, grad_out):
        xc, wc = ctx.saved_tensors
        g = grad_out.to(ctx.cdt).contiguous()
        gx = gw = gb = None
        if ctx.needs_input_grad[0]:
            gx = torch.matmul(g, wc).to(ctx.x_dtype)
        if ctx.needs_input_grad[1] or (ctx.has_bias and ctx.needs_input_grad[2]):
            gw, gb = token_wgrad(g, xc.contiguous(), want_bias=ctx.has_bias)
        return gx, gw, gb, None


def linear_tokens(x: torch.Tensor, weight: torch.Tensor, bias: torch.Tensor | None) -> torch.Tensor:
    amp = torch.is_autocast_enabled("cuda")
    bf16 = amp and torch.get_autocast_dtype("cuda") == torch.bfloat16
    if (torch.is_grad_enabled() and x.is_cuda and weight.requires_grad and weight.dtype == torch.float32
            and (bf16 or (not amp and x.dtype == torch.float32))
            and weight.shape[0] % 8 == 0 and weight.shape[1] % 8 == 0
            and x.numel() // weight.shape[1] * max(weight.shape) * (2 if bf16 else 4) < 0x7fffffff):
        with torch.autocast("cuda", enabled=False):
            return _TokenLinear.apply(x, weight, bias, bf16)
    return torch.nn.functional.linear(x, weight, bias)
```

Before: 288.0.

## Add wide 128-bit epilogue stores to split conv kernels via transposed MFMA

Result: no change. 290.4, median of 6 (+0.8%).

```diff
diff --git a/include/wm2f.h b/include/wm2f.h
--- a/include/wm2f.h
+++ b/include/wm2f.h
@@ -174,6 +174,12 @@
                            int Wi, int stride, int relu, int config, void* stream);
 int wm2f_conv3x3_split_config(int N, int P, int B, int n_cu);
 
+int wm2f_conv_split_wide_io(const void* x, const void* residual, const void* out, int64_t P);
+int wm2f_conv1x1_split_fwd_io(const void* x, const void* w_split, const void* bias, const void* residual, void* out, int B,
+                              int K, int N, int Hi, int Wi, int stride, int relu, int config, int io, void* stream);
+int wm2f_conv3x3_split_fwd_io(const void* x, const void* w_split, const void* bias, void* out, int B, int Cin, int N, int Hi,
+                              int Wi, int stride, int relu, int config, int io, void* stream);
+
 int wm2f_stem7x7_pool_fwd(const void* x, const void* w_split, const void* bias, void* out, int B, int Cin, int N, int Hi,
                           int Wi, int grid, void* stream);
 
diff --git a/weed_instance_segmentation_amd/_lib.py b/weed_instance_segmentation_amd/_lib.py
--- a/weed_instance_segmentation_amd/_lib.py
+++ b/weed_instance_segmentation_amd/_lib.py
@@ -102,6 +102,9 @@
     "wm2f_conv1x1_split_fwd": (c_int, [_P, _P, _P, _P, _P, _I, _I, _I, _I, _I, _I, _I, _I, _P]),
     "wm2f_conv3x3_split_config": (c_int, [_I, _I, _I, _I]),
     "wm2f_conv3x3_split_fwd": (c_int, [_P, _P, _P, _P, _I, _I, _I, _I, _I, _I, _I, _I, _P]),
+    "wm2f_conv_split_wide_io": (c_int, [_P, _P, _P, c_int64]),
+    "wm2f_conv1x1_split_fwd_io": (c_int, [_P, _P, _P, _P, _P, _I, _I, _I, _I, _I, _I, _I, _I, _I, _P]),
+    "wm2f_conv3x3_split_fwd_io": (c_int, [_P, _P, _P, _P, _I, _I, _I, _I, _I, _I, _I, _I, _I, _P]),
     "wm2f_stem7x7_pool_fwd": (c_int, [_P, _P, _P, _P, _I, _I, _I, _I, _I, _I, _P]),
     "wm2f_token_wgrad_workspace": (c_int64, [c_int64, _I, _I]),
     "wm2f_token_wgrad_bf16": (c_int, [_P, _P, _P, _P, _P, c_int64, _I, _I, _P]),
diff --git a/weed_instance_segmentation_amd/csrc/conv1x1_split.hip b/weed_instance_segmentation_amd/csrc/conv1x1_split.hip
--- a/weed_instance_segmentation_amd/csrc/conv1x1_split.hip
+++ b/weed_instance_segmentation_amd/csrc/conv1x1_split.hip
@@ -5,6 +5,7 @@
 
 using f32x4 = __attribute__((ext_vector_type(4))) float;
 using f32x8 = __attribute__((ext_vector_type(8))) float;
+using u32x4 = __attribute__((ext_vector_type(4))) unsigned;
 using bf16x8 = __attribute__((ext_vector_type(8))) __bf16;
 typedef __attribute__((address_space(3))) void* lds_ptr_t;
 
@@ -17,6 +18,9 @@
 constexpr float kBf16Max = 3.38953139e38f;
 
 enum : int { kRaw = 0, kBias = 1, kBiasRelu = 2, kBiasResRelu = 3 };
+enum : int { kIoAuto = 0, kIoNarrow = 1, kIoWide = 2 };
+constexpr int64_t kWideStoreMaxP = 65536;
+enum : int { kAblStores = 1, kAblLoads = 2, kAblMfma = 4 };
 
 __device__ __forceinline__ void split3(const f32x8 x, bf16x8& h, bf16x8& m, bf16x8& l) {
   f32x8 xc;
@@ -43,7 +47,7 @@
   asm volatile("" ::: "memory");
 }
 
-template <int NRT, int WN, int EPI>
+template <int NRT, int WN, int EPI, bool WIDE, int ABL = 0>
 __global__ __launch_bounds__(kThreads) void conv1x1_split_kernel(C1Args a) {
   extern __shared__ __attribute__((aligned(16))) unsigned char smem[];
   constexpr int kRowTiles = WN * NRT;
@@ -108,13 +112,22 @@
 #pragma unroll
       for (int p = 0; p < 3; ++p) dst[p] = *reinterpret_cast<const bf16x8*>(panel + (rt * 3 + p) * kFrag + lane * 16);
     };
+    auto mm = [&](const bf16x8 w, const bf16x8 x, const f32x4 c) {
+      return WIDE ? __builtin_amdgcn_mfma_f32_16x16x32_bf16(x, w, c, 0, 0, 0) : __builtin_amdgcn_mfma_f32_16x16x32_bf16(w, x, c, 0, 0, 0);
+    };
     auto six = [&](f32x4 acc_in, const bf16x8 (&av)[3], int cc) {
-      f32x4 c = __builtin_amdgcn_mfma_f32_16x16x32_bf16(av[1], bm[cc], (f32x4){0.f, 0.f, 0.f, 0.f}, 0, 0, 0);
-      c = __builtin_amdgcn_mfma_f32_16x16x32_bf16(av[2], bh[cc], c, 0, 0, 0);
-      c = __builtin_amdgcn_mfma_f32_16x16x32_bf16(av[0], bl[cc], c, 0, 0, 0);
-      c = __builtin_amdgcn_mfma_f32_16x16x32_bf16(av[1], bh[cc], c, 0, 0, 0);
-      c = __builtin_amdgcn_mfma_f32_16x16x32_bf16(av[0], bm[cc], c, 0, 0, 0);
-      return acc_in + __builtin_amdgcn_mfma_f32_16x16x32_bf16(av[0], bh[cc], c, 0, 0, 0);
+      if (ABL & kAblMfma) {
+        acc_in[0] += __builtin_bit_cast(f32x4, av[0])[0] * __builtin_bit_cast(f32x4, bl[cc])[0];
+        acc_in[1] += __builtin_bit_cast(f32x4, av[1])[1] * __builtin_bit_cast(f32x4, bm[cc])[1];
+        acc_in[2] += __builtin_bit_cast(f32x4, av[2])[2] * __builtin_bit_cast(f32x4, bh[cc])[2];
+        return acc_in;
+      }
+      f32x4 c = mm(av[1], bm[cc], (f32x4){0.f, 0.f, 0.f, 0.f});
+      c = mm(av[2], bh[cc], c);
+      c = mm(av[0], bl[cc], c);
+      c = mm(av[1], bh[cc], c);
+      c = mm(av[0], bm[cc], c);
+      return acc_in + mm(av[0], bh[cc], c);
     };
     bf16x8 av[2][3];
     read_a(av[0], 0);
@@ -133,6 +146,69 @@
   const __amdgpu_buffer_rsrc_t o_rs = __builtin_amdgcn_make_buffer_rsrc((void*)(a.out + img), 0, a.N * a.P * 4, 0x00020000);
   __amdgpu_buffer_rsrc_t r_rs = o_rs;
   if (EPI == kBiasResRelu) r_rs = __builtin_amdgcn_make_buffer_rsrc((void*)(a.residual + img), 0, a.N * a.P * 4, 0x00020000);
+  const bool st = !(ABL & kAblStores) || a.P < 0;
+  constexpr bool kLoadRes = EPI == kBiasResRelu && !(ABL & kAblLoads);
+
+  if (WIDE) {
+    const int n0 = n_wg + wn * NRT * 16 + j;
+    float bv[NRT];
+#pragma unroll
+    for (int rt = 0; rt < NRT; ++rt) bv[rt] = EPI != kRaw ? a.bias[n0 + rt * 16] : 0.f;
+    unsigned ro[kCT];
+#pragma unroll
+    for (int c = 0; c < kCT; ++c) {
+      const int p = p_w + c * 16 + 4 * g;
+      ro[c] = p < a.P ? (unsigned)((n0 * a.P + p) * 4) : kOob;
+    }
+    const unsigned rs = (unsigned)a.P * 64;
+    auto row = [&](int c, int rt) { return ro[c] == kOob ? kOob : ro[c] + (unsigned)rt * rs; };
+    auto finish = [&](f32x4 v, const float bias, const f32x4 res) {
+#pragma unroll
+      for (int e = 0; e < 4; ++e) {
+        if (EPI != kRaw) v[e] += bias;
+        if (EPI == kBiasResRelu) v[e] += res[e];
+        if (EPI == kBiasRelu || EPI == kBiasResRelu) v[e] = v[e] < 0.f ? 0.f : v[e];
+      }
+      return v;
+    };
+    const f32x4 zero4 = {0.f, 0.f, 0.f, 0.f};
+    if (kLoadRes) {
+      constexpr int kRB = NRT >= 8 ? 4 : 2;
+      f32x4 rv[2][kRB][kCT];
+      auto load_batch = [&](int h0, f32x4 (&dst)[kRB][kCT]) {
+#pragma unroll
+        for (int i = 0; i < kRB; ++i)
+#pragma unroll
+          for (int c = 0; c < kCT; ++c)
+            dst[i][c] = __builtin_bit_cast(f32x4, __builtin_amdgcn_raw_buffer_load_b128(r_rs, ro[c], (h0 + i) * rs, 0));
+      };
+      load_batch(0, rv[0]);
+#pragma unroll
+      for (int h0 = 0; h0 < NRT; h0 += kRB) {
+        const int cur = (h0 / kRB) & 1;
+        if (h0 + kRB < NRT) load_batch(h0 + kRB, rv[cur ^ 1]);
+        __builtin_amdgcn_sched_barrier(0);
+#pragma unroll
+        for (int i = 0; i < kRB; ++i)
+#pragma unroll
+          for (int c = 0; c < kCT; ++c) {
+            const f32x4 v = finish(acc[h0 + i][c], bv[h0 + i], rv[cur][i][c]);
+            if (st) __builtin_amdgcn_raw_buffer_store_b128(__builtin_bit_cast(u32x4, v), o_rs, row(c, h0 + i), 0, 0);
+          }
+        __builtin_amdgcn_sched_barrier(0);
+      }
+    } else {
+#pragma unroll
+      for (int rt = 0; rt < NRT; ++rt)
+#pragma unroll
+        for (int c = 0; c < kCT; ++c) {
+          const f32x4 v = finish(acc[rt][c], bv[rt], zero4);
+          if (st) __builtin_amdgcn_raw_buffer_store_b128(__builtin_bit_cast(u32x4, v), o_rs, row(c, rt), 0, 0);
+        }
+    }
+    return;
+  }
+
   const int n0 = n_wg + wn * NRT * 16 + 4 * g;
 #pragma unroll
   for (int rt = 0; rt < NRT; ++rt) {
@@ -147,7 +223,7 @@
       const unsigned ro = p < a.P ? (unsigned)(((n0 + rt * 16) * a.P + p) * 4) : kOob;
       const unsigned rs = (unsigned)a.P * 4;
       float rv[4] = {0.f, 0.f, 0.f, 0.f};
-      if (EPI == kBiasResRelu) {
+      if (kLoadRes) {
 #pragma unroll
         for (int e = 0; e < 4; ++e) rv[e] = __builtin_bit_cast(float, __builtin_amdgcn_raw_buffer_load_b32(r_rs, ro, e * rs, 0));
       }
@@ -157,7 +233,7 @@
         if (EPI != kRaw) v += bv[e];
         if (EPI == kBiasResRelu) v += rv[e];
         if (EPI == kBiasRelu || EPI == kBiasResRelu) v = v < 0.f ? 0.f : v;
-        __builtin_amdgcn_raw_buffer_store_b32(__builtin_bit_cast(unsigned, v), o_rs, ro, e * rs, 0);
+        if (st) __builtin_amdgcn_raw_buffer_store_b32(__builtin_bit_cast(unsigned, v), o_rs, ro, e * rs, 0);
       }
     }
   }
@@ -169,23 +245,24 @@
 constexpr Cfg kCfg[] = {{16, 1}, {8, 2}, {4, 4}, {8, 1}, {4, 1}};
 constexpr int kNumCfg = sizeof(kCfg) / sizeof(kCfg[0]);
 
-template <int NRT, int WN>
+template <int NRT, int WN, bool WIDE, int ABL>
 void (*pick_epi(int epi))(C1Args) {
   switch (epi) {
-    case kRaw: return conv1x1_split_kernel<NRT, WN, kRaw>;
-    case kBias: return conv1x1_split_kernel<NRT, WN, kBias>;
-    case kBiasRelu: return conv1x1_split_kernel<NRT, WN, kBiasRelu>;
-    default: return conv1x1_split_kernel<NRT, WN, kBiasResRelu>;
-  }
-}
-
+    case kRaw: return conv1x1_split_kernel<NRT, WN, kRaw, WIDE, ABL>;
+    case kBias: return conv1x1_split_kernel<NRT, WN, kBias, WIDE, ABL>;
+    case kBiasRelu: return conv1x1_split_kernel<NRT, WN, kBiasRelu, WIDE, ABL>;
+    default: return conv1x1_split_kernel<NRT, WN, kBiasResRelu, WIDE, ABL>;
+  }
+}
+
+template <bool WIDE, int ABL = 0>
 void (*pick_kernel(int ci, int epi))(C1Args) {
   switch (ci) {
-    case 0: return pick_epi<16, 1>(epi);
-    case 1: return pick_epi<8, 2>(epi);
-    case 2: return pick_epi<4, 4>(epi);
-    case 3: return pick_epi<8, 1>(epi);
-    default: return pick_epi<4, 1>(epi);
+    case 0: return pick_epi<16, 1, WIDE, ABL>(epi);
+    case 1: return pick_epi<8, 2, WIDE, ABL>(epi);
+    case 2: return pick_epi<4, 4, WIDE, ABL>(epi);
+    case 3: return pick_epi<8, 1, WIDE, ABL>(epi);
+    default: return pick_epi<4, 1, WIDE, ABL>(epi);
   }
 }
 
@@ -226,9 +303,15 @@
   return choose_cfg(N, P, B, n_cu);
 }
 
-extern "C" int wm2f_conv1x1_split_fwd(const void* x, const void* w_split, const void* bias, const void* residual, void* out,
-                                      int B, int K, int N, int Hi, int Wi, int stride, int relu, int config, void* stream) {
-  const char* who = "wm2f_conv1x1_split_fwd";
+extern "C" int wm2f_conv_split_wide_io(const void* x, const void* residual, const void* out, int64_t P) {
+  const uintptr_t bits = (uintptr_t)x | (uintptr_t)residual | (uintptr_t)out;
+  return P > 0 && P % 4 == 0 && bits % 16 == 0;
+}
+
+namespace {
+
+int conv1x1_run(const char* who, const void* x, const void* w_split, const void* bias, const void* residual, void* out, int B,
+                int K, int N, int Hi, int Wi, int stride, int relu, int config, int io, void* stream) {
   WM2F_REQUIRE(x && w_split && out, "%s: null pointer", who);
   WM2F_REQUIRE(B > 0 && K > 0 && N > 0 && Hi > 0 && Wi > 0, "%s: non-positive size", who);
   WM2F_REQUIRE(K % kKStep == 0 && N % 64 == 0, "%s: K = %d must be a multiple of %d and N = %d of 64", who, K, kKStep, N);
@@ -240,6 +323,16 @@
   WM2F_REQUIRE((int64_t)N * K * 6 < (1ll << 31), "%s: the split weight must stay below 2 GiB", who);
   WM2F_REQUIRE(!residual || (bias && relu), "%s: the residual epilogue is bias + residual + ReLU", who);
   WM2F_REQUIRE(!relu || bias, "%s: the ReLU epilogues carry a bias", who);
+  if (residual) {
+    const int64_t bytes = (int64_t)B * N * P * 4;
+    const char *r0 = (const char*)residual, *o0 = (const char*)out;
+    WM2F_REQUIRE(r0 + bytes <= o0 || o0 + bytes <= r0, "%s: residual and out overlap", who);
+  }
+  WM2F_REQUIRE(io == kIoAuto || io == kIoNarrow || io == kIoWide, "%s: io = %d (0 auto, 1 narrow, 2 wide)", who, io);
+  const bool can_wide = wm2f_conv_split_wide_io(x, residual, out, P) != 0;
+  WM2F_REQUIRE(io != kIoWide || can_wide,
+               "%s: the wide store form needs Ho * Wo = %lld a multiple of 4 and x, residual, out 16-byte aligned", who, (long long)P);
+  bool wide = io == kIoWide || (io == kIoAuto && can_wide && (residual || P < kWideStoreMaxP));
   int n_cu = 0;
   if (cu_count(&n_cu) != 0) {
     set_error("%s: cannot query the device", who);
@@ -264,7 +357,20 @@
   a.P = (int)P;
   a.stride = stride;
   const size_t lds = (size_t)2 * (nt / 16) * 3 * kFrag;
-  void (*kfn)(C1Args) = pick_kernel(ci, epi);
+  void (*kfn)(C1Args) = wide ? pick_kernel<true>(ci, epi) : pick_kernel<false>(ci, epi);
+#ifdef WM2F_PROFILING
+  {
+    const char* ea = getenv("WM2F_C1_ABL");
+    const int abl = ea ? atoi(ea) : 0;
+    if (abl != 0) {
+      WM2F_REQUIRE(abl == 1 || abl == 2 || abl == 3 || abl == 4, "%s: WM2F_C1_ABL = %d is not built (1, 2, 3, 4 are)", who, abl);
+      WM2F_REQUIRE(io != kIoWide, "%s: WM2F_C1_ABL ablates the narrow kernel only", who);
+      wide = false;
+      kfn = abl == 1 ? pick_kernel<false, 1>(ci, epi)
+                     : (abl == 2 ? pick_kernel<false, 2>(ci, epi) : (abl == 3 ? pick_kernel<false, 3>(ci, epi) : pick_kernel<false, 4>(ci, epi)));
+    }
+  }
+#endif
   hipError_t e = hipFuncSetAttribute((const void*)kfn, hipFuncAttributeMaxDynamicSharedMemorySize, (int)lds);
   if (e != hipSuccess) {
     set_error("%s: cannot raise dynamic LDS to %zu: %s", who, lds, hipGetErrorString(e));
@@ -274,3 +380,18 @@
   WM2F_CHECK_LAUNCH(who);
   return WM2F_OK;
 }
+
+}
+
+extern "C" int wm2f_conv1x1_split_fwd_io(const void* x, const void* w_split, const void* bias, const void* residual, void* out,
+                                         int B, int K, int N, int Hi, int Wi, int stride, int relu, int config, int io,
+                                         void* stream) {
+  return conv1x1_run("wm2f_conv1x1_split_fwd_io", x, w_split, bias, residual, out, B, K, N, Hi, Wi, stride, relu, config, io,
+                     stream);
+}
+
+extern "C" int wm2f_conv1x1_split_fwd(const void* x, const void* w_split, const void* bias, const void* residual, void* out,
+                                      int B, int K, int N, int Hi, int Wi, int stride, int relu, int config, void* stream) {
+  return conv1x1_run("wm2f_conv1x1_split_fwd", x, w_split, bias, residual, out, B, K, N, Hi, Wi, stride, relu, config, kIoAuto,
+                     stream);
+}
diff --git a/weed_instance_segmentation_amd/csrc/conv3x3_split.hip b/weed_instance_segmentation_amd/csrc/conv3x3_split.hip
--- a/weed_instance_segmentation_amd/csrc/conv3x3_split.hip
+++ b/weed_instance_segmentation_amd/csrc/conv3x3_split.hip
@@ -5,6 +5,7 @@
 
 using f32x4 = __attribute__((ext_vector_type(4))) float;
 using f32x8 = __attribute__((ext_vector_type(8))) float;
+using u32x4 = __attribute__((ext_vector_type(4))) unsigned;
 using bf16x8 = __attribute__((ext_vector_type(8))) __bf16;
 typedef __attribute__((address_space(3))) void* lds_ptr_t;
 
@@ -17,6 +18,8 @@
 constexpr float kBf16Max = 3.38953139e38f;
 
 enum : int { kRaw = 0, kBias = 1, kBiasRelu = 2 };
+enum : int { kIoAuto = 0, kIoNarrow = 1, kIoWide = 2 };
+constexpr int64_t kWideStoreMaxP = 65536;
 
 __device__ __forceinline__ f32x8 widen(const bf16x8 v) {
   using u32x4 = __attribute__((ext_vector_type(4))) unsigned;
@@ -55,7 +58,7 @@
   asm volatile("" ::: "memory");
 }
 
-template <int NRT, int WN, int EPI>
+template <int NRT, int WN, int EPI, bool WIDE>
 __global__ __launch_bounds__(kThreads) void conv3x3_split_kernel(C3Args a) {
   extern __shared__ __attribute__((aligned(16))) unsigned char smem[];
   constexpr int kRowTiles = WN * NRT;
@@ -134,13 +137,16 @@
 #pragma unroll
       for (int p = 0; p < 3; ++p) dst[p] = *reinterpret_cast<const bf16x8*>(panel + (rt * 3 + p) * kFrag + lane * 16);
     };
+    auto mm = [&](const bf16x8 w, const bf16x8 x, const f32x4 c) {
+      return WIDE ? __builtin_amdgcn_mfma_f32_16x16x32_bf16(x, w, c, 0, 0, 0) : __builtin_amdgcn_mfma_f32_16x16x32_bf16(w, x, c, 0, 0, 0);
+    };
     auto six = [&](f32x4 acc_in, const bf16x8 (&av)[3], int cc) {
-      f32x4 c = __builtin_amdgcn_mfma_f32_16x16x32_bf16(av[1], bm[cc], (f32x4){0.f, 0.f, 0.f, 0.f}, 0, 0, 0);
-      c = __builtin_amdgcn_mfma_f32_16x16x32_bf16(av[2], bh[cc], c, 0, 0, 0);
-      c = __builtin_amdgcn_mfma_f32_16x16x32_bf16(av[0], bl[cc], c, 0, 0, 0);
-      c = __builtin_amdgcn_mfma_f32_16x16x32_bf16(av[1], bh[cc], c, 0, 0, 0);
-      c = __builtin_amdgcn_mfma_f32_16x16x32_bf16(av[0], bm[cc], c, 0, 0, 0);
-      return acc_in + __builtin_amdgcn_mfma_f32_16x16x32_bf16(av[0], bh[cc], c, 0, 0, 0);
+      f32x4 c = mm(av[1], bm[cc], (f32x4){0.f, 0.f, 0.f, 0.f});
+      c = mm(av[2], bh[cc], c);
+      c = mm(av[0], bl[cc], c);
+      c = mm(av[1], bh[cc], c);
+      c = mm(av[0], bm[cc], c);
+      return acc_in + mm(av[0], bh[cc], c);
     };
     bf16x8 av[2][3];
     read_a(av[0], 0);
@@ -157,6 +163,31 @@
 
   const int64_t img = (int64_t)b * a.N * a.P;
   const __amdgpu_buffer_rsrc_t o_rs = __builtin_amdgcn_make_buffer_rsrc((void*)(a.out + img), 0, a.N * a.P * 4, 0x00020000);
+
+  if (WIDE) {
+    const int n0 = n_wg + wn * NRT * 16 + j;
+    float bv[NRT];
+#pragma unroll
+    for (int rt = 0; rt < NRT; ++rt) bv[rt] = EPI != kRaw ? a.bias[n0 + rt * 16] : 0.f;
+    const unsigned rs = (unsigned)a.P * 64;
+#pragma unroll
+    for (int c = 0; c < kCT; ++c) {
+      const int p = p_w + c * 16 + 4 * g;
+      const unsigned ro = p < a.P ? (unsigned)((n0 * a.P + p) * 4) : kOob;
+#pragma unroll
+      for (int rt = 0; rt < NRT; ++rt) {
+        f32x4 v = acc[rt][c];
+#pragma unroll
+        for (int e = 0; e < 4; ++e) {
+          if (EPI != kRaw) v[e] += bv[rt];
+          if (EPI == kBiasRelu) v[e] = v[e] < 0.f ? 0.f : v[e];
+        }
+        __builtin_amdgcn_raw_buffer_store_b128(__builtin_bit_cast(u32x4, v), o_rs, ro == kOob ? kOob : ro + (unsigned)rt * rs, 0, 0);
+      }
+    }
+    return;
+  }
+
   const int n0 = n_wg + wn * NRT * 16 + 4 * g;
 #pragma unroll
   for (int rt = 0; rt < NRT; ++rt) {
@@ -187,22 +218,23 @@
 constexpr Cfg kCfg[] = {{16, 1}, {8, 2}, {4, 4}, {8, 1}, {4, 1}};
 constexpr int kNumCfg = sizeof(kCfg) / sizeof(kCfg[0]);
 
-template <int NRT, int WN>
+template <int NRT, int WN, bool WIDE>
 void (*pick_epi(int epi))(C3Args) {
   switch (epi) {
-    case kRaw: return conv3x3_split_kernel<NRT, WN, kRaw>;
-    case kBias: return conv3x3_split_kernel<NRT, WN, kBias>;
-    default: return conv3x3_split_kernel<NRT, WN, kBiasRelu>;
-  }
-}
-
+    case kRaw: return conv3x3_split_kernel<NRT, WN, kRaw, WIDE>;
+    case kBias: return conv3x3_split_kernel<NRT, WN, kBias, WIDE>;
+    default: return conv3x3_split_kernel<NRT, WN, kBiasRelu, WIDE>;
+  }
+}
+
+template <bool WIDE>
 void (*pick_kernel(int ci, int epi))(C3Args) {
   switch (ci) {
-    case 0: return pick_epi<16, 1>(epi);
-    case 1: return pick_epi<8, 2>(epi);
-    case 2: return pick_epi<4, 4>(epi);
-    case 3: return pick_epi<8, 1>(epi);
-    default: return pick_epi<4, 1>(epi);
+    case 0: return pick_epi<16, 1, WIDE>(epi);
+    case 1: return pick_epi<8, 2, WIDE>(epi);
+    case 2: return pick_epi<4, 4, WIDE>(epi);
+    case 3: return pick_epi<8, 1, WIDE>(epi);
+    default: return pick_epi<4, 1, WIDE>(epi);
   }
 }
 
@@ -243,9 +275,10 @@
   return choose_cfg(N, P, B, n_cu);
 }
 
-extern "C" int wm2f_conv3x3_split_fwd(const void* x, const void* w_split, const void* bias, void* out, int B, int Cin, int N,
-                                      int Hi, int Wi, int stride, int relu, int config, void* stream) {
-  const char* who = "wm2f_conv3x3_split_fwd";
+namespace {
+
+int conv3x3_run(const char* who, const void* x, const void* w_split, const void* bias, void* out, int B, int Cin, int N, int Hi,
+                int Wi, int stride, int relu, int config, int io, void* stream) {
   WM2F_REQUIRE(x && w_split && out, "%s: null pointer", who);
   WM2F_REQUIRE(B > 0 && Cin > 0 && N > 0 && Hi > 0 && Wi > 0, "%s: non-positive size", who);
   WM2F_REQUIRE(Cin % kKStep == 0 && N % 64 == 0, "%s: Cin = %d must be a multiple of %d and N = %d of 64", who, Cin, kKStep, N);
@@ -256,6 +289,11 @@
                "%s: one image of x / out must stay below 2 GiB (32-bit buffer offsets)", who);
   WM2F_REQUIRE((int64_t)N * 9 * Cin * 6 < (1ll << 31), "%s: the split weight must stay below 2 GiB", who);
   WM2F_REQUIRE(!relu || bias, "%s: the ReLU epilogue carries a bias", who);
+  WM2F_REQUIRE(io == kIoAuto || io == kIoNarrow || io == kIoWide, "%s: io = %d (0 auto, 1 narrow, 2 wide)", who, io);
+  const bool can_wide = wm2f_conv_split_wide_io(x, nullptr, out, P) != 0;
+  WM2F_REQUIRE(io != kIoWide || can_wide,
+               "%s: the wide store form needs Ho * Wo = %lld a multiple of 4 and x, out 16-byte aligned", who, (long long)P);
+  const bool wide = io == kIoWide || (io == kIoAuto && can_wide && P < kWideStoreMaxP);
   int n_cu = 0;
   if (cu_count(&n_cu) != 0) {
     set_error("%s: cannot query the device", who);
@@ -279,7 +317,7 @@
   a.P = (int)P;
   a.stride = stride;
   const size_t lds = (size_t)2 * (nt / 16) * 3 * kFrag;
-  void (*kfn)(C3Args) = pick_kernel(ci, epi);
+  void (*kfn)(C3Args) = wide ? pick_kernel<true>(ci, epi) : pick_kernel<false>(ci, epi);
   hipError_t e = hipFuncSetAttribute((const void*)kfn, hipFuncAttributeMaxDynamicSharedMemorySize, (int)lds);
   if (e != hipSuccess) {
     set_error("%s: cannot raise dynamic LDS to %zu: %s", who, lds, hipGetErrorString(e));
@@ -289,3 +327,15 @@
   WM2F_CHECK_LAUNCH(who);
   return WM2F_OK;
 }
+
+}
+
+extern "C" int wm2f_conv3x3_split_fwd_io(const void* x, const void* w_split, const void* bias, void* out, int B, int Cin, int N,
+                                         int Hi, int Wi, int stride, int relu, int config, int io, void* stream) {
+  return conv3x3_run("wm2f_conv3x3_split_fwd_io", x, w_split, bias, out, B, Cin, N, Hi, Wi, stride, relu, config, io, stream);
+}
+
+extern "C" int wm2f_conv3x3_split_fwd(const void* x, const void* w_split, const void* bias, void* out, int B, int Cin, int N,
+                                      int Hi, int Wi, int stride, int relu, int config, void* stream) {
+  return conv3x3_run("wm2f_conv3x3_split_fwd", x, w_split, bias, out, B, Cin, N, Hi, Wi, stride, relu, config, kIoAuto, stream);
+}
diff --git a/weed_instance_segmentation_amd/ops/__init__.py b/weed_instance_segmentation_amd/ops/__init__.py
--- a/weed_instance_segmentation_amd/ops/__init__.py
+++ b/weed_instance_segmentation_amd/ops/__init__.py
@@ -11,7 +11,7 @@
 from .ccl import label_components, resize_nearest_tables
 from .fused import (add_broadcast, bias_act_, bias_relu_maxpool, group_norm_act_, group_norm_tokens_, resize_bilinear,
                     resize_pyramid, tokens_to_nchw)
-from .gemm import (conv1x1, conv1x1_applies, conv3x3, conv3x3_applies, linear_tokens, split_weight, split_weight_3x3,
+from .gemm import (conv1x1, conv1x1_applies, conv1x1_io, conv3x3, conv3x3_applies, conv3x3_io, conv_wide_io, linear_tokens, split_weight, split_weight_3x3,
                    split_weight_cached, split_weight_stem, stem_conv_pool, stem_conv_pool_applies, stem_weight_columns,
                    stem_weight_matrix, token_linear, token_linear_applies, token_wgrad, token_wgrad_applies)
 from .k1 import (k1_bwd_deterministic, k1_lane_order, k1_lane_rows, k1_lanes_applies, k1_rows_applies, ms_deform_attn,
diff --git a/weed_instance_segmentation_amd/ops/gemm.py b/weed_instance_segmentation_amd/ops/gemm.py
--- a/weed_instance_segmentation_amd/ops/gemm.py
+++ b/weed_instance_segmentation_amd/ops/gemm.py
@@ -87,6 +87,20 @@
     return (out, out_pos) if pos is not None else out
 
 
+_CONV_IO = {"auto": 0, "narrow": 1, "wide": 2}
+
+
+def _conv_io(io: str, who: str) -> int:
+    if io not in _CONV_IO:
+        raise ValueError(f"{who}: io = {io!r} (auto, narrow, wide)")
+    return _CONV_IO[io]
+
+
+def conv_wide_io(x: torch.Tensor, out: torch.Tensor, residual: torch.Tensor | None = None) -> bool:
+    P = int(out.shape[-1]) * int(out.shape[-2])
+    return bool(load().wm2f_conv_split_wide_io(_p(x), _p(residual), _p(out), P))
+
+
 def conv1x1_applies(x: torch.Tensor, weight: torch.Tensor, stride: int = 1) -> bool:
     if x.dim() != 4 or weight.dim() not in (2, 4) or (weight.dim() == 4 and weight.shape[2:] != (1, 1)):
         return False
@@ -101,6 +115,13 @@
 def conv1x1(x: torch.Tensor, weight: torch.Tensor, bias: torch.Tensor | None = None, residual: torch.Tensor | None = None,
             relu: bool = False, stride: int = 1, split: bool = True, w_split: torch.Tensor | None = None,
             config: int = -1) -> torch.Tensor:
+    return conv1x1_io(x, weight, bias, residual, relu, stride, split, w_split, config, io="auto")
+
+
+def conv1x1_io(x: torch.Tensor, weight: torch.Tensor, bias: torch.Tensor | None = None, residual: torch.Tensor | None = None,
+               relu: bool = False, stride: int = 1, split: bool = True, w_split: torch.Tensor | None = None,
+               config: int = -1, io: str = "auto") -> torch.Tensor:
+    io_code = _conv_io(io, "conv1x1")
     if residual is not None and (bias is None or not relu):
         raise ValueError("conv1x1: the residual epilogue is bias + residual + ReLU")
     if relu and bias is None:
@@ -134,8 +155,8 @@
     elif w_split.dtype != torch.uint8 or w_split.numel() != N * K * 6 or w_split.device != x.device:
         raise ValueError("conv1x1: w_split is not split_weight(weight)")
     out = torch.empty(B, N, Ho, Wo, device=x.device, dtype=torch.float32)
-    _launch("wm2f_conv1x1_split_fwd", x, _p(x), _p(w_split), _p(bias), _p(residual), _p(out), B, K, N, H, W, int(stride),
-            1 if relu else 0, int(config), tag=f"conv1x1_K{K}_N{N}_P{Ho * Wo}")
+    _launch("wm2f_conv1x1_split_fwd_io", x, _p(x), _p(w_split), _p(bias), _p(residual), _p(out), B, K, N, H, W, int(stride),
+            1 if relu else 0, int(config), io_code, tag=f"conv1x1_K{K}_N{N}_P{Ho * Wo}")
     return out
 
 
@@ -152,6 +173,12 @@
 
 def conv3x3(x: torch.Tensor, weight: torch.Tensor, bias: torch.Tensor | None = None, relu: bool = False, stride: int = 1,
             split: bool = True, w_split: torch.Tensor | None = None, config: int = -1) -> torch.Tensor:
+    return conv3x3_io(x, weight, bias, relu, stride, split, w_split, config, io="auto")
+
+
+def conv3x3_io(x: torch.Tensor, weight: torch.Tensor, bias: torch.Tensor | None = None, relu: bool = False, stride: int = 1,
+               split: bool = True, w_split: torch.Tensor | None = None, config: int = -1, io: str = "auto") -> torch.Tensor:
+    io_code = _conv_io(io, "conv3x3")
     if relu and bias is None:
         raise ValueError("conv3x3: the ReLU epilogue carries a bias")
     if not split or not conv3x3_applies(x, weight, stride):
@@ -175,8 +202,8 @@
     elif w_split.dtype != torch.uint8 or w_split.numel() != N * 9 * Cin * 6 or w_split.device != x.device:
         raise ValueError("conv3x3: w_split is not split_weight_3x3(weight)")
     out = torch.empty(B, N, Ho, Wo, device=x.device, dtype=torch.float32)
-    _launch("wm2f_conv3x3_split_fwd", x, _p(x), _p(w_split), _p(bias), _p(out), B, Cin, N, H, W, int(stride), 1 if relu else 0,
-            int(config), tag=f"conv3x3_C{Cin}_N{N}_P{Ho * Wo}")
+    _launch("wm2f_conv3x3_split_fwd_io", x, _p(x), _p(w_split), _p(bias), _p(out), B, Cin, N, H, W, int(stride),
+            1 if relu else 0, int(config), io_code, tag=f"conv3x3_C{Cin}_N{N}_P{Ho * Wo}")
     return out
 
 
```
